# Ghostish/Open3DSOT

Hardware: NVIDIA H100
Metric: template-search pairs/sec, BAT-Car fwd+bwd (higher is better)
Workload: dtype f32

## Files before the change

### open3dsot_b200/csrc/common.cuh

```cuda
#pragma once
#include <cuda_runtime.h>
#include <stdint.h>

#define O3D_OK 0
#define O3D_ERR_ARG (-1)
#define O3D_ERR_ALIGN (-2)
#define O3D_ERR_CUDA (-3)

void o3d_set_error(const char* fmt, ...);

#define O3D_REQUIRE(cond, code, ...)                 \
    do {                                             \
        if (!(cond)) {                               \
            o3d_set_error(__VA_ARGS__);              \
            return (code);                           \
        }                                            \
    } while (0)

#define O3D_CHECK_LAUNCH(name)                                                        \
    do {                                                                              \
        cudaError_t e__ = cudaGetLastError();                                         \
        if (e__ != cudaSuccess) {                                                     \
            o3d_set_error("%s: launch failed: %s", name, cudaGetErrorString(e__));    \
            return O3D_ERR_CUDA;                                                      \
        }                                                                             \
    } while (0)

#define O3D_CUDA(call, name)                                                          \
    do {                                                                              \
        cudaError_t e__ = (call);                                                     \
        if (e__ != cudaSuccess) {                                                     \
            o3d_set_error("%s: %s", name, cudaGetErrorString(e__));                   \
            return O3D_ERR_CUDA;                                                      \
        }                                                                             \
    } while (0)

static inline int o3d_num_sms() {
    static int sms = 0;
    if (sms == 0) {
        int dev = 0;
        cudaGetDevice(&dev);
        cudaDeviceGetAttribute(&sms, cudaDevAttrMultiProcessorCount, dev);
        if (sms <= 0) sms = 132;
    }
    return sms;
}

static inline int o3d_opt_n_threads(int work) {
    if (work < 1) return 1;
    int p = 0;
    while ((1 << (p + 1)) <= work) ++p;
    int t = 1 << p;
    return t > 512 ? 512 : t;
}

#ifdef __CUDACC__
__device__ __forceinline__ float o3d_sq3(float dx, float dy, float dz) {
    return __fmaf_rn(dz, dz, __fmaf_rn(dy, dy, __fmul_rn(dx, dx)));
}
__device__ __forceinline__ float o3d_dist2(float ax, float ay, float az, float bx, float by, float bz) {
    return o3d_sq3(__fsub_rn(ax, bx), __fsub_rn(ay, by), __fsub_rn(az, bz));
}

__device__ __forceinline__ uint32_t o3d_smem_u32(const void* p) {
    return static_cast<uint32_t>(__cvta_generic_to_shared(p));
}
__device__ __forceinline__ void o3d_mbar_init(uint64_t* bar, uint32_t count) {
    asm volatile("mbarrier.init.shared::cta.b64 [%0], %1;" ::"r"(o3d_smem_u32(bar)), "r"(count));
}
__device__ __forceinline__ void o3d_fence_mbar_init() {
    asm volatile("fence.mbarrier_init.release.cluster;" ::: "memory");
}
__device__ __forceinline__ void o3d_fence_proxy_async() {
    asm volatile("fence.proxy.async.shared::cta;" ::: "memory");
}
__device__ __forceinline__ void o3d_mbar_expect_tx(uint64_t* bar, uint32_t bytes) {
    asm volatile("mbarrier.arrive.expect_tx.shared::cta.b64 _, [%0], %1;" ::"r"(o3d_smem_u32(bar)), "r"(bytes)
                 : "memory");
}
__device__ __forceinline__ void o3d_mbar_arrive(uint64_t* bar) {
    asm volatile("mbarrier.arrive.shared::cta.b64 _, [%0];" ::"r"(o3d_smem_u32(bar)) : "memory");
}
__device__ __forceinline__ bool o3d_mbar_try_wait(uint64_t* bar, uint32_t parity) {
    uint32_t ok;
    asm volatile(
        "{\n\t.reg .pred p;\n\t"
        "mbarrier.try_wait.parity.shared::cta.b64 p, [%1], %2;\n\t"
        "selp.u32 %0, 1, 0, p;\n\t}"
        : "=r"(ok)
        : "r"(o3d_smem_u32(bar)), "r"(parity)
        : "memory");
    return ok != 0;
}
__device__ __forceinline__ void o3d_mbar_wait(uint64_t* bar, uint32_t parity) {
    for (uint32_t spin = 0; spin < (1u << 28); ++spin)
        if (o3d_mbar_try_wait(bar, parity)) return;
    __trap();
}
__device__ __forceinline__ void o3d_bulk_g2s(void* smem_dst, const void* gsrc, uint32_t bytes, uint64_t* bar) {
    asm volatile(
        "cp.async.bulk.shared::cluster.global.mbarrier::complete_tx::bytes [%0], [%1], %2, [%3];" ::"r"(
            o3d_smem_u32(smem_dst)),
        "l"(gsrc), "r"(bytes), "r"(o3d_smem_u32(bar))
        : "memory");
}
__device__ __forceinline__ void o3d_prefetch_l2(const void* gptr, size_t bytes) {
    const char* p = static_cast<const char*>(gptr);
    const uintptr_t a = reinterpret_cast<uintptr_t>(p);
    const uintptr_t lo = a & ~(uintptr_t)15;
    size_t n = ((a - lo) + bytes + 15) & ~(size_t)15;
    const char* q = reinterpret_cast<const char*>(lo);
    while (n > 0) {
        const uint32_t c = n > (1u << 20) ? (1u << 20) : (uint32_t)n;
        asm volatile("cp.async.bulk.prefetch.L2.global [%0], %1;" ::"l"(q), "r"(c) : "memory");
        q += c;
        n -= c;
    }
}
__device__ __forceinline__ uint32_t o3d_block_exscan1024(uint32_t v, uint32_t* s_warp, uint32_t& total) {
    const int lane = threadIdx.x & 31, warp = threadIdx.x >> 5;
    uint32_t inc = v;
#pragma unroll
    for (int o = 1; o < 32; o <<= 1) {
        const uint32_t t = __shfl_up_sync(0xFFFFFFFFu, inc, o);
        if (lane >= o) inc += t;
    }
    if (lane == 31) s_warp[warp] = inc;
    __syncthreads();
    uint32_t w = s_warp[lane];
    uint32_t winc = w;
#pragma unroll
    for (int o = 1; o < 32; o <<= 1) {
        const uint32_t t = __shfl_up_sync(0xFFFFFFFFu, winc, o);
        if (lane >= o) winc += t;
    }
    total = __shfl_sync(0xFFFFFFFFu, winc, 31);
    const uint32_t wbase = __shfl_sync(0xFFFFFFFFu, winc - w, warp);
    __syncthreads();
    return wbase + inc - v;
}
__device__ __forceinline__ void o3d_to_box_frame(float dx, float dy, float dz, const float (&R)[9], float& x, float& y, float& z) {
    x = fmaf(dz, R[6], fmaf(dy, R[3], dx * R[0]));
    y = fmaf(dz, R[7], fmaf(dy, R[4], dx * R[1]));
    z = fmaf(dz, R[8], fmaf(dy, R[5], dx * R[2]));
}
__device__ __forceinline__ uint32_t o3d_lanemask_lt() {
    uint32_t m;
    asm("mov.u32 %0, %%lanemask_lt;" : "=r"(m));
    return m;
}
int o3d_pw_fwd_tc_dir(const float* x, int ldx, const float* in_scale, const float* in_shift, int in_relu, const void* wtiles,
                      const float* bias, int P, int K, int N, float* y, int ldy, double* sum, double* sumsq, int S, float* ymax,
                      float* ymin, int32_t* arg, int ldp, void* stream, bool reverse, bool bf16);
struct o3d_lift_t;
int o3d_pw_fwd_tc_lift_prec(const o3d_lift_t* lf, const int32_t* gidx, const float* in_scale, const float* in_shift, int in_relu,
                            const void* wtiles, const float* bias, int P, int K, int N, float* y, int ldy, double* sum,
                            double* sumsq, int S, float* ymax, float* ymin, int32_t* arg, int ldp, void* stream, bool bf16);
int o3d_pw_dgrad_tc_prec(const float* g, int ldg, const float* y, int ldy, const float* a, const float* b, const float* cc,
                         const float* dpool, const int32_t* sel, int S, int ldp, const void* wtiles_t, int P, int Cout, int Cin,
                         float* out, int ldo, const float* yprev, int ldyp, const float* pscale, const float* pshift, int prelu,
                         double* s1, double* s2y, void* stream, bool bf16);
int o3d_pw_dgrad_tc_lift_prec(const float* g, int ldg, const float* y, int ldy, const float* a, const float* b, const float* cc,
                              const float* dpool, const int32_t* sel, int S, int ldp, const void* wtiles_t, int P, int Cout,
                              int Cin, float* out, int ldo, const o3d_lift_t* lf, const int32_t* gidx, const float* pscale,
                              const float* pshift, int prelu, double* s1, double* s2y, void* stream, bool bf16);
int o3d_pw_wgrad_tc2_prec(const float* g, int ldg, const float* y, int ldy, const float* a, const float* b, const float* cc,
                          const float* dpool, const int32_t* sel, int S, int ldp, const float* x, int ldx, const float* in_scale,
                          const float* in_shift, int in_relu, int P, int Cout, int Cin, float* dw, int lddw, float* part,
                          long long part_floats, void* stream, bool bf16);
int o3d_pw_wgrad_tc_lift_prec(const float* g, int ldg, const float* y, int ldy, const float* a, const float* b, const float* cc,
                              const float* dpool, const int32_t* sel, int S, int ldp, const o3d_lift_t* lf, const int32_t* gidx,
                              const float* in_scale, const float* in_shift, int in_relu, int P, int Cout, int Cin, float* dw,
                              int lddw, float* part, long long part_floats, void* stream, bool bf16);
int o3d_pw_bwd_tc_prec(const float* g, int ldg, const float* y, int ldy, const float* a, const float* b, const float* cc,
                       const float* dpool, const int32_t* sel, int S, int ldp, const void* wtiles_t, const float* x,
                       const o3d_lift_t* lf, const int32_t* gidx, const float* in_scale, const float* in_shift, int in_relu, int P,
                       int Cout, int Cin, float* out, double* s1, double* s2y, float* dw, int lddw, float* part,
                       long long part_floats, void* stream, bool bf16);

#endif
```

### open3dsot_b200/csrc/lift.cu

```cuda
#include "common.cuh"
#include "lift.cuh"
#include "../../include/o3d_b200.h"

namespace {

constexpr int LIFT_THREADS = 256;

__device__ __forceinline__ float4 ldg4(const float* p) { return __ldg(reinterpret_cast<const float4*>(p)); }

struct LiftGeom { const int32_t* ridx; int ridx_mod, rows_per_cloud, pos_per_cloud; };

__device__ __forceinline__ int lift_row(const LiftGeom& g, int p) {
    const int cloud = p / g.pos_per_cloud;
    const int local = g.ridx ? __ldg(g.ridx + p) : (p % g.ridx_mod);
    return cloud * g.rows_per_cloud + local;
}

struct U4 { float4 u0, u1, u2, u3; };
__device__ __forceinline__ U4 load_u(const LiftView& lv, int c) {
    const float4 z = make_float4(0.f, 0.f, 0.f, 0.f);
    if (!lv.u) return U4{z, z, z, z};
    return U4{ldg4(lv.u + c), ldg4(lv.u + lv.ldz + c), ldg4(lv.u + 2 * lv.ldz + c), ldg4(lv.u + 3 * lv.ldz + c)};
}

template <bool STORE>
__global__ void __launch_bounds__(LIFT_THREADS, 4)
    lift_stats_kernel(LiftView lv, LiftGeom geo, int P, int C0, int grp, int32_t* __restrict__ gidx, float* __restrict__ y0,
                      double* __restrict__ sum, double* __restrict__ sumsq) {
    extern __shared__ double red[];
    const int tpr = C0 >> 2, rl = blockDim.x / tpr;
    const int t = threadIdx.x % tpr, lane = threadIdx.x / tpr;
    const int c = t * 4;
    const int n_groups = P / grp;
    const U4 u = load_u(lv, c);
    const float4 zero = make_float4(0.f, 0.f, 0.f, 0.f);
    if (!STORE && !sum) {
        if (lv.z && t == 0)
            for (int g = blockIdx.x * rl + lane; g < n_groups; g += gridDim.x * rl)
                for (int s = 0; s < grp; ++s) gidx[g * grp + s] = lift_row(geo, g * grp + s);
        return;
    }
    double d1[4] = {0.0, 0.0, 0.0, 0.0}, d2[4] = {0.0, 0.0, 0.0, 0.0};
    for (int g = blockIdx.x * rl + lane; g < n_groups; g += gridDim.x * rl) {
        float4 a1 = zero, a2 = zero;
        const int pb = g * grp;
#pragma unroll 4
        for (int s = 0; s < grp; ++s) {
            const int p = pb + s;
            float4 z4 = zero;
            if (lv.z) {
                const int row = lift_row(geo, p);
                if (t == 0) gidx[p] = row;
                z4 = ldg4(lv.z + (size_t)row * lv.ldz + c);
            }
            const float4 sv = lv.s ? ldg4(lv.s + (size_t)p * 4) : zero;
            const float4 v = lift_val4(z4, sv, u.u0, u.u1, u.u2, u.u3);
            if (STORE) *reinterpret_cast<float4*>(y0 + (size_t)p * lv.ldz + c) = v;
            a1.x += v.x; a1.y += v.y; a1.z += v.z; a1.w += v.w;
            a2.x = fmaf(v.x, v.x, a2.x); a2.y = fmaf(v.y, v.y, a2.y); a2.z = fmaf(v.z, v.z, a2.z); a2.w = fmaf(v.w, v.w, a2.w);
            if ((s & 31) == 31 || s == grp - 1) {
                d1[0] += a1.x; d1[1] += a1.y; d1[2] += a1.z; d1[3] += a1.w;
                d2[0] += a2.x; d2[1] += a2.y; d2[2] += a2.z; d2[3] += a2.w;
                a1 = a2 = zero;
            }
        }
    }
    if (!sum) return;
#pragma unroll
    for (int j = 0; j < 4; ++j) {
        red[(size_t)lane * C0 + c + j] = d1[j];
        red[(size_t)(rl + lane) * C0 + c + j] = d2[j];
    }
    __syncthreads();
    for (int ch = threadIdx.x; ch < C0; ch += blockDim.x) {
        double s1 = 0.0, s2 = 0.0;
        for (int l = 0; l < rl; ++l) { s1 += red[(size_t)l * C0 + ch]; s2 += red[(size_t)(rl + l) * C0 + ch]; }
        atomicAdd(sum + ch, s1);
        atomicAdd(sumsq + ch, s2);
    }
}

__global__ void __launch_bounds__(LIFT_THREADS, 4)
    lift_scatter_kernel(LiftView lv, int P, int C0, int grp, const float* __restrict__ y0, const float* __restrict__ g, int ldg,
                        const float* __restrict__ ca, const float* __restrict__ cb, const float* __restrict__ ccf,
                        float* __restrict__ dz, float* __restrict__ ds, float* __restrict__ du) {
    extern __shared__ float redf[];
    const int tpr = C0 >> 2, rl = blockDim.x / tpr;
    const int t = threadIdx.x % tpr, lane = threadIdx.x / tpr;
    const int c = t * 4;
    const int n_groups = P / grp;
    const U4 u = load_u(lv, c);
    const float4 one = make_float4(1.f, 1.f, 1.f, 1.f), zero = make_float4(0.f, 0.f, 0.f, 0.f);
    const float4 a4 = ca ? ldg4(ca + c) : one, b4 = ca ? ldg4(cb + c) : zero, k4 = ca ? ldg4(ccf + c) : zero;
    float4 du0 = zero, du1 = zero, du2 = zero, du3 = zero;
    const int w = tpr >= 32 ? 32 : tpr;
    const bool shfl = (tpr <= 32 && (tpr & (tpr - 1)) == 0) || (tpr % 32 == 0);
    for (int gb = blockIdx.x * rl; gb < n_groups; gb += gridDim.x * rl) {
        const bool valid = gb + lane < n_groups;
        const int gi = valid ? gb + lane : n_groups - 1;
        float4 acc0 = zero;
        const int pb = gi * grp;
        const int row0 = lv.z ? __ldg(lv.gidx + pb) : 0;
#pragma unroll 4
        for (int s = 0; s < grp; ++s) {
            const int p = pb + s;
            const int row = lv.z ? __ldg(lv.gidx + p) : 0;
            const float4 g4 = ldg4(g + (size_t)p * ldg + c);
            const float4 sv = lv.s ? ldg4(lv.s + (size_t)p * 4) : zero;
            float4 dy = g4;
            if (ca) {
                float4 v;
                if (y0) v = ldg4(y0 + (size_t)p * lv.ldz + c);
                else v = lift_val4(lv.z ? ldg4(lv.z + (size_t)row * lv.ldz + c) : zero, sv, u.u0, u.u1, u.u2, u.u3);
                dy.x = fmaf(a4.x, g4.x, fmaf(k4.x, v.x, b4.x)); dy.y = fmaf(a4.y, g4.y, fmaf(k4.y, v.y, b4.y));
                dy.z = fmaf(a4.z, g4.z, fmaf(k4.z, v.z, b4.z)); dy.w = fmaf(a4.w, g4.w, fmaf(k4.w, v.w, b4.w));
            }
            if (dz) {
                if (row == row0) { acc0.x += dy.x; acc0.y += dy.y; acc0.z += dy.z; acc0.w += dy.w; }
                else if (valid) atomicAdd(reinterpret_cast<float4*>(dz + (size_t)row * lv.ldz + c), dy);
            }
            if (du && valid) {
                du0.x = fmaf(sv.x, dy.x, du0.x); du0.y = fmaf(sv.x, dy.y, du0.y); du0.z = fmaf(sv.x, dy.z, du0.z); du0.w = fmaf(sv.x, dy.w, du0.w);
                du1.x = fmaf(sv.y, dy.x, du1.x); du1.y = fmaf(sv.y, dy.y, du1.y); du1.z = fmaf(sv.y, dy.z, du1.z); du1.w = fmaf(sv.y, dy.w, du1.w);
                du2.x = fmaf(sv.z, dy.x, du2.x); du2.y = fmaf(sv.z, dy.y, du2.y); du2.z = fmaf(sv.z, dy.z, du2.z); du2.w = fmaf(sv.z, dy.w, du2.w);
                du3.x = fmaf(sv.w, dy.x, du3.x); du3.y = fmaf(sv.w, dy.y, du3.y); du3.z = fmaf(sv.w, dy.z, du3.z); du3.w = fmaf(sv.w, dy.w, du3.w);
            }
            if (ds) {
                float4 d;
                d.x = fmaf(dy.x, u.u0.x, fmaf(dy.y, u.u0.y, fmaf(dy.z, u.u0.z, dy.w * u.u0.w)));
                d.y = fmaf(dy.x, u.u1.x, fmaf(dy.y, u.u1.y, fmaf(dy.z, u.u1.z, dy.w * u.u1.w)));
                d.z = fmaf(dy.x, u.u2.x, fmaf(dy.y, u.u2.y, fmaf(dy.z, u.u2.z, dy.w * u.u2.w)));
                d.w = fmaf(dy.x, u.u3.x, fmaf(dy.y, u.u3.y, fmaf(dy.z, u.u3.z, dy.w * u.u3.w)));
                if (shfl) {
                    for (int o = w >> 1; o >= 1; o >>= 1) {
                        d.x += __shfl_xor_sync(0xFFFFFFFFu, d.x, o, 32); d.y += __shfl_xor_sync(0xFFFFFFFFu, d.y, o, 32);
                        d.z += __shfl_xor_sync(0xFFFFFFFFu, d.z, o, 32); d.w += __shfl_xor_sync(0xFFFFFFFFu, d.w, o, 32);
                    }
                    if ((t & (w - 1)) == 0 && valid) atomicAdd(reinterpret_cast<float4*>(ds + (size_t)p * 4), d);
                } else if (valid) {
                    atomicAdd(reinterpret_cast<float4*>(ds + (size_t)p * 4), d);
                }
            }
        }
        if (dz && valid) atomicAdd(reinterpret_cast<float4*>(dz + (size_t)row0 * lv.ldz + c), acc0);
    }
    if (!du) return;
    float* r = redf + (size_t)lane * 4 * C0 + c;
    *reinterpret_cast<float4*>(r) = du0;
    *reinterpret_cast<float4*>(r + C0) = du1;
    *reinterpret_cast<float4*>(r + 2 * C0) = du2;
    *reinterpret_cast<float4*>(r + 3 * C0) = du3;
    __syncthreads();
    for (int e = threadIdx.x; e < 4 * C0; e += blockDim.x) {
        float s1 = 0.f;
        for (int l = 0; l < rl; ++l) s1 += redf[(size_t)l * 4 * C0 + e];
        atomicAdd(du + e, s1);
    }
}

int lift_check(const o3d_lift_t* lf, int P, int C0, const char* who) {
    O3D_REQUIRE(lf && (lf->z || lf->s), O3D_ERR_ARG, "%s: null lift descriptor (need z and / or s)", who);
    O3D_REQUIRE(C0 >= 4 && (C0 & 3) == 0 && C0 <= 1024 && lf->ldz == C0, O3D_ERR_ARG, "%s: C0=%d ldz=%d (need C0 %% 4 == 0, ldz == C0)",
                who, C0, lf->ldz);
    O3D_REQUIRE(lf->grp >= 1 && (lf->grp & (lf->grp - 1)) == 0 && P % lf->grp == 0, O3D_ERR_ARG,
                "%s: grp=%d must be a power of two dividing P=%d", who, lf->grp, P);
    O3D_REQUIRE(!lf->z || (lf->pos_per_cloud >= 1 && lf->rows_per_cloud >= 1 && (lf->ridx || lf->ridx_mod >= 1)), O3D_ERR_ARG,
                "%s: bad cloud geometry", who);
    O3D_REQUIRE(((uintptr_t)lf->s & 15) == 0 && ((uintptr_t)lf->u & 15) == 0 && ((uintptr_t)lf->z & 15) == 0, O3D_ERR_ALIGN,
                "%s: z / s / u must be 16-byte aligned", who);
    O3D_REQUIRE((lf->s == nullptr) == (lf->u == nullptr), O3D_ERR_ARG, "%s: s and u come together", who);
    return O3D_OK;
}

inline LiftView make_view(const o3d_lift_t* lf, const int32_t* gidx) {
    return LiftView{lf->z, lf->ldz, lf->z ? gidx : nullptr, lf->s, lf->u};
}

inline void lift_launch_shape(int P, int C0, int grp, int& threads, int& blocks, int& rl) {
    const int tpr = C0 / 4;
    rl = LIFT_THREADS / tpr;
    if (rl < 1) rl = 1;
    threads = tpr * rl;
    const int n_groups = P / grp;
    blocks = (n_groups + rl - 1) / rl;
    const int cap = 8 * o3d_num_sms();
    if (blocks > cap) blocks = cap;
    if (blocks < 1) blocks = 1;
}

}

extern "C" int o3d_lift_stats(const o3d_lift_t* lf, int P, int C0, int32_t* gidx, float* y0, double* sum, double* sumsq,
                              void* stream) {
    if (int e = lift_check(lf, P, C0, "o3d_lift_stats")) return e;
    O3D_REQUIRE(gidx || !lf->z, O3D_ERR_ARG, "o3d_lift_stats: gidx workspace missing");
    if (P == 0 || (!lf->z && !y0 && !sum)) return O3D_OK;
    int threads, blocks, rl;
    lift_launch_shape(P, C0, lf->grp, threads, blocks, rl);
    const LiftView lv = make_view(lf, gidx);
    const LiftGeom geo{lf->ridx, lf->ridx_mod, lf->rows_per_cloud, lf->pos_per_cloud};
    const size_t smem = sum ? sizeof(double) * 2 * rl * C0 : 0;
    cudaStream_t st = (cudaStream_t)stream;
    if (y0) lift_stats_kernel<true><<<blocks, threads, smem, st>>>(lv, geo, P, C0, lf->grp, gidx, y0, sum, sumsq);
    else lift_stats_kernel<false><<<blocks, threads, smem, st>>>(lv, geo, P, C0, lf->grp, gidx, y0, sum, sumsq);
    O3D_CHECK_LAUNCH("o3d_lift_stats");
    return O3D_OK;
}

extern "C" int o3d_lift_scatter(const o3d_lift_t* lf, int P, int C0, const int32_t* gidx, const float* y0, const float* g,
                                int ldg, const float* a, const float* b, const float* cc, void* stream) {
    if (int e = lift_check(lf, P, C0, "o3d_lift_scatter")) return e;
    O3D_REQUIRE((gidx || !lf->z) && g && (ldg & 3) == 0, O3D_ERR_ARG, "o3d_lift_scatter: null pointer / ldg");
    O3D_REQUIRE(!lf->d_s || lf->u, O3D_ERR_ARG, "o3d_lift_scatter: d_s without u");
    O3D_REQUIRE(((uintptr_t)lf->d_s & 15) == 0 && ((uintptr_t)lf->d_z & 15) == 0, O3D_ERR_ALIGN, "o3d_lift_scatter: alignment");
    if (P == 0) return O3D_OK;
    int threads, blocks, rl;
    lift_launch_shape(P, C0, lf->grp, threads, blocks, rl);
    const LiftView lv = make_view(lf, gidx);
    const size_t smem = (lf->s && lf->d_u) ? sizeof(float) * rl * 4 * C0 : 0;
    lift_scatter_kernel<<<blocks, threads, smem, (cudaStream_t)stream>>>(lv, P, C0, lf->grp, y0, g, ldg, a, b, cc,
                                                                        lf->z ? lf->d_z : nullptr, lf->s ? lf->d_s : nullptr,
                                                                        lf->s ? lf->d_u : nullptr);
    O3D_CHECK_LAUNCH("o3d_lift_scatter");
    return O3D_OK;
}
```

### open3dsot_b200/csrc/lift.cuh

```cuda
#pragma once
#include <stdint.h>

struct LiftView {
    const float* z; int ldz;
    const int32_t* gidx;
    const float* s;
    const float* u;
};

#ifdef __CUDACC__
__device__ __forceinline__ float lift_val(float z, const float4& s, float u0, float u1, float u2, float u3) {
    return fmaf(s.w, u3, fmaf(s.z, u2, fmaf(s.y, u1, fmaf(s.x, u0, z))));
}
__device__ __forceinline__ float4 lift_val4(const float4& z, const float4& s, const float4& u0, const float4& u1, const float4& u2,
                                            const float4& u3) {
    return make_float4(lift_val(z.x, s, u0.x, u1.x, u2.x, u3.x), lift_val(z.y, s, u0.y, u1.y, u2.y, u3.y),
                       lift_val(z.z, s, u0.z, u1.z, u2.z, u3.z), lift_val(z.w, s, u0.w, u1.w, u2.w, u3.w));
}
#endif
```

### open3dsot_b200/csrc/pwmlp_tc.cu

```cuda
#include <type_traits>
#include "common.cuh"
#include "lift.cuh"
#include "tc_ptx.cuh"
#include "../../include/o3d_b200.h"

namespace {

struct TcAct {
    const float* x; int ld; const float* scale; const float* shift; int relu;
    struct Coef { float4 s, t; bool on; };
    template <int R> struct Batch { float4 v[R]; };
    __device__ __forceinline__ Coef prep(int k, int K) const {
        Coef c;
        c.on = k < K;
        c.s = make_float4(1.f, 1.f, 1.f, 1.f);
        c.t = make_float4(0.f, 0.f, 0.f, 0.f);
        if (c.on && scale) { c.s = ld4g(scale + k); c.t = ld4g(shift + k); }
        return c;
    }
    template <int R>
    __device__ __forceinline__ void fetch(Batch<R>& b, int p0, int stride, int P, int k, int K) const {
        const int kk = k < K ? k : 0;
#pragma unroll
        for (int i = 0; i < R; ++i) {
            const int p = p0 + i * stride;
            b.v[i] = ld4g(x + (size_t)(p < P ? p : P - 1) * ld + kk);
        }
    }
    template <int R>
    __device__ __forceinline__ float4 finish(const Batch<R>& b, const Coef& c, int i, int p, int P) const {
        float4 v = b.v[i];
        if (!(c.on && p < P)) return make_float4(0.f, 0.f, 0.f, 0.f);
        if (scale) { v.x = fmaf(v.x, c.s.x, c.t.x); v.y = fmaf(v.y, c.s.y, c.t.y); v.z = fmaf(v.z, c.s.z, c.t.z); v.w = fmaf(v.w, c.s.w, c.t.w); }
        if (relu) { v.x = fmaxf(v.x, 0.f); v.y = fmaxf(v.y, 0.f); v.z = fmaxf(v.z, 0.f); v.w = fmaxf(v.w, 0.f); }
        return v;
    }
    __device__ __forceinline__ void prefetch_rows(int p0, int rows, int P) const {
        if (p0 < P) o3d_prefetch_l2(x + (size_t)p0 * ld, (size_t)min(rows, P - p0) * ld * sizeof(float));
    }
};

struct TcLift {
    LiftView lv; const float* scale; const float* shift; int relu;
    int la;
    struct Coef { float4 s, t, u0, u1, u2, u3; bool on; };
    template <int R> struct Batch { float4 v[R]; float4 sv[R]; int nrow[R]; int tag; };
    __device__ __forceinline__ Coef prep(int k, int K) const {
        Coef c;
        c.on = k < K;
        c.s = make_float4(1.f, 1.f, 1.f, 1.f);
        c.t = c.u0 = c.u1 = c.u2 = c.u3 = make_float4(0.f, 0.f, 0.f, 0.f);
        if (c.on && scale) { c.s = ld4g(scale + k); c.t = ld4g(shift + k); }
        if (c.on && lv.u) { c.u0 = ld4g(lv.u + k); c.u1 = ld4g(lv.u + lv.ldz + k); c.u2 = ld4g(lv.u + 2 * lv.ldz + k); c.u3 = ld4g(lv.u + 3 * lv.ldz + k); }
        return c;
    }
    template <int R>
    __device__ __forceinline__ void fetch(Batch<R>& b, int p0, int stride, int P, int k, int K) const {
        const int kk = k < K ? k : 0;
        if (lv.z) {
            int row[R];
            if (b.tag == p0 + 1) {
#pragma unroll
                for (int i = 0; i < R; ++i) row[i] = b.nrow[i];
            } else if (R == 4 && stride == 1 && (p0 & 3) == 0 && p0 + 3 < P) {
                const int4 r4 = __ldg(reinterpret_cast<const int4*>(lv.gidx + p0));
                row[0] = r4.x; row[R > 1 ? 1 : 0] = r4.y; row[R > 2 ? 2 : 0] = r4.z; row[R > 3 ? 3 : 0] = r4.w;
            } else {
#pragma unroll
                for (int i = 0; i < R; ++i) {
                    const int p = p0 + i * stride;
                    row[i] = __ldg(lv.gidx + (p < P ? p : P - 1));
                }
            }
#pragma unroll
            for (int i = 0; i < R; ++i) b.v[i] = ld4g(lv.z + (size_t)row[i] * lv.ldz + kk);
            if (la == 0) {
#pragma unroll
                for (int i = 0; i < R; ++i) b.nrow[i] = row[i];
                b.tag = p0 + 1;
            } else {
                const int pn = p0 + la;
#pragma unroll
                for (int i = 0; i < R; ++i) {
                    const int p = pn + i * stride;
                    b.nrow[i] = __ldg(lv.gidx + (p < P ? p : P - 1));
                }
                b.tag = pn + 1;
            }
        }
        if (lv.s) {
#pragma unroll
            for (int i = 0; i < R; ++i) {
                const int p = p0 + i * stride;
                b.sv[i] = ld4g(lv.s + (size_t)(p < P ? p : P - 1) * 4);
            }
        }
    }
    template <int R>
    __device__ __forceinline__ float4 finish(const Batch<R>& b, const Coef& c, int i, int p, int P) const {
        const float4 zero = make_float4(0.f, 0.f, 0.f, 0.f);
        if (!(c.on && p < P)) return zero;
        float4 v = lift_val4(lv.z ? b.v[i] : zero, lv.s ? b.sv[i] : zero, c.u0, c.u1, c.u2, c.u3);
        if (scale) { v.x = fmaf(v.x, c.s.x, c.t.x); v.y = fmaf(v.y, c.s.y, c.t.y); v.z = fmaf(v.z, c.s.z, c.t.z); v.w = fmaf(v.w, c.s.w, c.t.w); }
        if (relu) { v.x = fmaxf(v.x, 0.f); v.y = fmaxf(v.y, 0.f); v.z = fmaxf(v.z, 0.f); v.w = fmaxf(v.w, 0.f); }
        return v;
    }
    __device__ __forceinline__ void prefetch_rows(int p0, int rows, int P) const {
        if (p0 >= P) return;
        const size_t n = (size_t)min(rows, P - p0);
        if (lv.z) o3d_prefetch_l2(lv.gidx + p0, n * sizeof(int32_t));
        if (lv.s) o3d_prefetch_l2(lv.s + (size_t)p0 * 4, n * 16);
    }
};

struct TcDy {
    const float* g; int ldg; const float* y; int ldy; const float* a; const float* b; const float* cc;
    const float* dpool; const int32_t* sel; int S; int ldp;
    int sh;
    struct Coef { float4 a, b, c; bool on; };
    template <int R> struct Batch { float4 g[R]; float4 y[R]; bool shared; };
    __device__ __forceinline__ Coef prep(int k, int K) const {
        Coef c;
        c.on = k < K;
        c.a = make_float4(1.f, 1.f, 1.f, 1.f);
        c.b = c.c = make_float4(0.f, 0.f, 0.f, 0.f);
        if (c.on && a) { c.a = ld4g(a + k); c.b = ld4g(b + k); c.c = ld4g(cc + k); }
        return c;
    }
    template <int R>
    __device__ __forceinline__ void fetch(Batch<R>& bt, int p0, int stride, int P, int k, int K) const {
        const int kk = k < K ? k : 0;
        bt.shared = false;
        if (dpool) {
            const int pf = p0 < P ? p0 : P - 1;
            const int pe = p0 + (R - 1) * stride;
            const int pl = pe < P ? pe : P - 1;
            if (R >= 2 && (pf >> sh) == (pl >> sh)) {
                bt.shared = true;
                const size_t go = (size_t)(pf >> sh) * ldp + kk;
                bt.g[0] = ld4g(dpool + go);
                const int4 sl = __ldg(reinterpret_cast<const int4*>(sel + go));
                bt.g[R >= 2 ? 1 : 0] = make_float4(__int_as_float(sl.x), __int_as_float(sl.y), __int_as_float(sl.z), __int_as_float(sl.w));
            } else {
#pragma unroll
                for (int i = 0; i < R; ++i) {
                    const int p = p0 + i * stride, pp = p < P ? p : P - 1;
                    const int s = pp & (S - 1);
                    const size_t go = (size_t)(pp >> sh) * ldp + kk;
                    const int4 sl = __ldg(reinterpret_cast<const int4*>(sel + go));
                    const float4 d = ld4g(dpool + go);
                    bt.g[i] = make_float4(sl.x == s ? d.x : 0.f, sl.y == s ? d.y : 0.f, sl.z == s ? d.z : 0.f, sl.w == s ? d.w : 0.f);
                }
            }
        } else {
#pragma unroll
            for (int i = 0; i < R; ++i) {
                const int p = p0 + i * stride;
                bt.g[i] = ld4g(g + (size_t)(p < P ? p : P - 1) * ldg + kk);
            }
        }
#pragma unroll
        for (int i = 0; i < R; ++i) {
            const int p = p0 + i * stride;
            bt.y[i] = a ? ld4g(y + (size_t)(p < P ? p : P - 1) * ldy + kk) : make_float4(0.f, 0.f, 0.f, 0.f);
        }
    }
    template <int R>
    __device__ __forceinline__ float4 finish(const Batch<R>& bt, const Coef& c, int i, int p, int P) const {
        if (!(c.on && p < P)) return make_float4(0.f, 0.f, 0.f, 0.f);
        float4 v = bt.g[i];
        if (bt.shared) {
            const int s = p & (S - 1);
            const float4 d = bt.g[0], sl = bt.g[R >= 2 ? 1 : 0];
            v = make_float4(__float_as_int(sl.x) == s ? d.x : 0.f, __float_as_int(sl.y) == s ? d.y : 0.f,
                            __float_as_int(sl.z) == s ? d.z : 0.f, __float_as_int(sl.w) == s ? d.w : 0.f);
        }
        if (a) {
            const float4 yy = bt.y[i];
            v.x = fmaf(c.a.x, v.x, fmaf(c.c.x, yy.x, c.b.x)); v.y = fmaf(c.a.y, v.y, fmaf(c.c.y, yy.y, c.b.y));
            v.z = fmaf(c.a.z, v.z, fmaf(c.c.z, yy.z, c.b.z)); v.w = fmaf(c.a.w, v.w, fmaf(c.c.w, yy.w, c.b.w));
        }
        return v;
    }
    __device__ __forceinline__ void prefetch_rows(int p0, int rows, int P) const {
        if (p0 >= P) return;
        const size_t n = (size_t)min(rows, P - p0);
        if (!dpool) o3d_prefetch_l2(g + (size_t)p0 * ldg, n * ldg * sizeof(float));
        if (a) o3d_prefetch_l2(y + (size_t)p0 * ldy, n * ldy * sizeof(float));
        if (dpool) {
            const int g0 = p0 >> sh, g1 = (p0 + (int)n - 1) >> sh;
            const size_t bytes = (size_t)(g1 - g0 + 1) * ldp * sizeof(float);
            o3d_prefetch_l2(dpool + (size_t)g0 * ldp, bytes);
            o3d_prefetch_l2(sel + (size_t)g0 * ldp, bytes);
        }
    }
};

template <class L> struct Bf16 : L {};
template <class L> struct is_bf16 { static constexpr bool value = false; };
template <class L> struct is_bf16<Bf16<L>> { static constexpr bool value = true; };
template <class L> struct is_lift { static constexpr bool value = std::is_same<L, TcLift>::value; };
template <class L> struct is_lift<Bf16<L>> { static constexpr bool value = is_lift<L>::value; };

template <int LD>
struct TcFwdEpi {
    float* y; int ldy; const float* bias; double* sum; double* sumsq;
    int S, log2S; float* ymax; float* ymin; int32_t* arg; int ldp;
    float bv, mx, mn; int ax, an; double d1, d2;
    __device__ __forceinline__ void begin(int ch, int Nw) {
        d1 = d2 = 0.0;
        bv = (bias && ch < Nw) ? bias[ch] : 0.f;
        mx = -INFINITY; mn = INFINITY; ax = an = 0;
    }
    __device__ __forceinline__ void prefetch(int, int, int, int) {}
    __device__ __forceinline__ const int32_t* lift_gidx() const { return nullptr; }
    __device__ __forceinline__ const float* lift_s() const { return nullptr; }
    __device__ __forceinline__ void set_tile(const int32_t*, const float4*) {}
    __device__ __forceinline__ void group(const uint32_t (&r)[16], int ch, int Nw, int pbase, int P) {
        if (ch >= Nw) return;
        float s1 = 0.f, s2 = 0.f;
        const int smask = S - 1;
        float* yp = y ? y + (size_t)pbase * ldy + ch : nullptr;
        if (pbase + 16 <= P && (S == 0 || S >= 16)) {
            float v[16];
#pragma unroll
            for (int j = 0; j < 16; ++j) v[j] = __uint_as_float(r[j]) + bv;
            if (yp) {
                const size_t st = LD ? (size_t)LD : (size_t)ldy;
#pragma unroll
                for (int j = 0; j < 16; ++j) yp[j * st] = v[j];
            }
#pragma unroll
            for (int j = 0; j < 16; ++j) {
                s1 += v[j];
                s2 = fmaf(v[j], v[j], s2);
            }
            if (S > 0) {
                float gm = v[0], gn = v[0];
                int ga = 0, gb = 0;
#pragma unroll
                for (int j = 1; j < 16; ++j) {
                    if (v[j] > gm) { gm = v[j]; ga = j; }
                    if (v[j] < gn) { gn = v[j]; gb = j; }
                }
                const int s0 = pbase & smask;
                if (s0 == 0) { mx = gm; ax = ga; mn = gn; an = gb; }
                else {
                    if (gm > mx) { mx = gm; ax = s0 + ga; }
                    if (gn < mn) { mn = gn; an = s0 + gb; }
                }
                if (s0 + 16 == S) {
                    const size_t o = (size_t)(pbase >> log2S) * ldp + ch;
                    ymax[o] = mx; ymin[o] = mn; arg[o] = ax | (an << 16);
                }
            }
        } else {
#pragma unroll
            for (int j = 0; j < 16; ++j) {
                if (pbase + j >= P) break;
                const float v = __uint_as_float(r[j]) + bv;
                if (yp) yp[(size_t)j * ldy] = v;
                s1 += v;
                s2 = fmaf(v, v, s2);
                if (S > 0) {
                    const int s = (pbase + j) & smask;
                    if (s == 0) { mx = -INFINITY; mn = INFINITY; ax = an = 0; }
                    if (v > mx) { mx = v; ax = s; }
                    if (v < mn) { mn = v; an = s; }
                    if (s == smask) {
                        const size_t o = (size_t)((pbase + j) >> log2S) * ldp + ch;
                        ymax[o] = mx; ymin[o] = mn; arg[o] = ax | (an << 16);
                    }
                }
            }
        }
        d1 += (double)s1;
        d2 += (double)s2;
    }
    __device__ __forceinline__ void end(int ch, int Nw) {
        if (sum && ch < Nw) {
            atomicAdd(sum + ch, d1);
            atomicAdd(sumsq + ch, d2);
        }
    }
};

template <int LD, bool LIFT = false>
struct TcDgradEpi {
    float* out; int ldo; const float* yprev; int ldyp; const float* scale; const float* shift; int relu;
    double* s1g; double* s2y;
    LiftView lv;
    float sc, sh; double d1, d2;
    float yv[16];
    float u0, u1, u2, u3; const int32_t* gs; const float4* ss;
    __device__ __forceinline__ bool lifted() const { return LIFT; }
    __device__ __forceinline__ void begin(int ch, int Nw) {
        d1 = d2 = 0.0;
        sc = (scale && ch < Nw) ? scale[ch] : 1.f;
        sh = (shift && ch < Nw) ? shift[ch] : 0.f;
        if constexpr (LIFT) {
            const bool on = lv.u && ch < Nw;
            u0 = on ? lv.u[ch] : 0.f; u1 = on ? lv.u[lv.ldz + ch] : 0.f; u2 = on ? lv.u[2 * lv.ldz + ch] : 0.f; u3 = on ? lv.u[3 * lv.ldz + ch] : 0.f;
            gs = nullptr;
        }
    }
    __device__ __forceinline__ const int32_t* lift_gidx() const { return LIFT ? lv.gidx : nullptr; }
    __device__ __forceinline__ const float* lift_s() const { return LIFT ? lv.s : nullptr; }
    __device__ __forceinline__ void set_tile(const int32_t* g, const float4* s4) { if constexpr (LIFT) { gs = g; ss = s4; } }
    __device__ __forceinline__ void prefetch_lift(int ch, int pbase, int col, int P) {
#pragma unroll
        for (int j = 0; j < 16; ++j) {
            const float z = lv.z ? __ldg(lv.z + (size_t)gs[col + j] * lv.ldz + ch) : 0.f;
            const float4 sv = lv.s ? ss[col + j] : make_float4(0.f, 0.f, 0.f, 0.f);
            yv[j] = lift_val(z, sv, u0, u1, u2, u3);
        }
    }
    __device__ __forceinline__ void prefetch(int ch, int Nw, int pbase, int P) {
        if (ch >= Nw) return;
        if constexpr (LIFT) { prefetch_lift(ch, pbase, pbase & (TC_N - 1), P); return; }
        if (!yprev) return;
        if (pbase + 16 <= P) {
            const float* yp = yprev + (size_t)pbase * ldyp + ch;
            const size_t st = LD ? (size_t)LD : (size_t)ldyp;
#pragma unroll
            for (int j = 0; j < 16; ++j) yv[j] = __ldg(yp + j * st);
        } else {
#pragma unroll
            for (int j = 0; j < 16; ++j) {
                const int pj = min(pbase + j, P - 1);
                yv[j] = __ldg(yprev + (size_t)pj * ldyp + ch);
            }
        }
    }
    __device__ __forceinline__ void group(const uint32_t (&r)[16], int ch, int Nw, int pbase, int P) {
        if (ch >= Nw) return;
        float s1 = 0.f, s2 = 0.f;
        float* op = out + (size_t)pbase * ldo + ch;
        if (pbase + 16 <= P) {
            float v[16];
#pragma unroll
            for (int j = 0; j < 16; ++j) v[j] = __uint_as_float(r[j]);
            if (yprev || lifted()) {
                if (relu) {
#pragma unroll
                    for (int j = 0; j < 16; ++j) v[j] = fmaf(yv[j], sc, sh) > 0.f ? v[j] : 0.f;
                }
#pragma unroll
                for (int j = 0; j < 16; ++j) s2 = fmaf(v[j], yv[j], s2);
            }
            const size_t st = LD ? (size_t)LD : (size_t)ldo;
#pragma unroll
            for (int j = 0; j < 16; ++j) {
                s1 += v[j];
                op[j * st] = v[j];
            }
        } else {
#pragma unroll
            for (int j = 0; j < 16; ++j) {
                if (pbase + j >= P) break;
                float v = __uint_as_float(r[j]);
                if (yprev || lifted()) {
                    if (relu && !(fmaf(yv[j], sc, sh) > 0.f)) v = 0.f;
                    s2 = fmaf(v, yv[j], s2);
                }
                s1 += v;
                op[(size_t)j * ldo] = v;
            }
        }
        d1 += (double)s1;
        d2 += (double)s2;
    }
    __device__ __forceinline__ void end(int ch, int Nw) {
        if (s1g && ch < Nw) {
            atomicAdd(s1g + ch, d1);
            atomicAdd(s2y + ch, d2);
        }
    }
};

constexpr int TC_STAGES = 2;
constexpr int TC_STAGE_BYTES = 4 * TILE_BYTES;
constexpr int TC_EPI_LD = 68;
constexpr int TC_EPI_BYTES = TC_M * TC_EPI_LD * 4;
constexpr int TC_THREADS = 512;
constexpr int TC_SMEM = TC_STAGES * TC_STAGE_BYTES + 2 * TC_EPI_BYTES + 1024 + 256 + 1024 + 4096;

template <int R>
__device__ __forceinline__ void stage_acc(const float (&acc)[R], float* stg, int ld) {
    const int w = (threadIdx.x >> 5) & 3, lane = threadIdx.x & 31;
#pragma unroll
    for (int i = 0; i < R; ++i) {
        const int row = 16 * w + (lane >> 2) + 8 * ((i >> 1) & 1), col = 8 * (i >> 2) + 2 * (lane & 3) + (i & 1);
        stg[col * ld + row] = acc[i];
    }
}

template <class BLoad, class Epi>
__global__ void __launch_bounds__(TC_THREADS, 1)
    pw_tc_kernel(BLoad bl, const uint8_t* __restrict__ wtiles, int P, int K, int Nw, int nkb, Epi epi, int rev) {
    constexpr bool BF = is_bf16<BLoad>::value;
    constexpr int WBYTES = BF ? BF_TILE_BYTES : 2 * TILE_BYTES;
    extern __shared__ uint8_t smem_raw[];
    uint8_t* smem = reinterpret_cast<uint8_t*>((reinterpret_cast<uintptr_t>(smem_raw) + 1023) & ~(uintptr_t)1023);
    uint8_t* tail = smem + TC_STAGES * TC_STAGE_BYTES + 2 * TC_EPI_BYTES;
    uint64_t* full = reinterpret_cast<uint64_t*>(tail);
    uint64_t* empty = full + TC_STAGES;

    const int warp = threadIdx.x >> 5, lane = threadIdx.x & 31;
    const int mt0 = blockIdx.y;
    const int n_ptiles = (P + TC_N - 1) / TC_N;
    auto tile_of = [&](int t) { return rev ? n_ptiles - 1 - t : t; };

    if (threadIdx.x == 0) {
        for (int s = 0; s < TC_STAGES; ++s) {
            o3d_mbar_init(full + s, 256 + 1);
            o3d_mbar_init(empty + s, 8);
        }
        o3d_fence_mbar_init();
    }
    __syncthreads();

    if (warp < 8) {
        const int h = warp >> 2;
        const int tw = threadIdx.x & 127;
        const int ch = mt0 * TC_M + tw;
        float* stg = reinterpret_cast<float*>(smem + TC_STAGES * TC_STAGE_BYTES + h * TC_EPI_BYTES);
        int32_t* gsm = reinterpret_cast<int32_t*>(tail + 256);
        float4* ssm = reinterpret_cast<float4*>(tail + 256 + 1024);
        epi.begin(ch, Nw);
        int stage = 0, phase = 0, buf = 0;
        for (int t = blockIdx.x; t < n_ptiles; t += gridDim.x) {
            const int pt0 = tile_of(t) * TC_N;
            {
                const int32_t* gi = epi.lift_gidx();
                const float* si = epi.lift_s();
                if (gi || si) {
                    const int pp = min(pt0 + tw, P - 1);
                    if (gi && h == 0) gsm[buf * TC_N + tw] = __ldg(gi + pp);
                    if (si && h == 1) ssm[buf * TC_N + tw] = ld4g(si + (size_t)pp * 4);
                    asm volatile("bar.sync 1, 256;" ::: "memory");
                    epi.set_tile(gsm + buf * TC_N, ssm + buf * TC_N);
                }
            }
            const int pb = pt0 + h * 64;
            epi.prefetch(ch, Nw, pb, P);
            float acc[64];
#pragma unroll
            for (int i = 0; i < 64; ++i) acc[i] = 0.f;
            for (int kb = 0; kb < nkb; ++kb) {
                o3d_mbar_wait(full + stage, phase);
                const uint32_t sb = o3d_smem_u32(smem + stage * TC_STAGE_BYTES);
                wgmma_fence_acc(acc);
                wgmma_fence();
                if constexpr (BF) {
                    const uint32_t xb = sb + 2 * TILE_BYTES + h * (BF_TILE_BYTES / 2);
                    wgmma_bf16_kblock<128>(acc, make_desc_sw64(xb), make_desc_sw64(sb), kb == 0);
                } else {
                    const uint32_t xb = sb + 2 * TILE_BYTES + h * (TILE_BYTES / 2);
                    wgmma_3xtf32_kblock<128>(acc, make_desc(xb), make_desc(xb + TILE_BYTES), make_desc(sb), make_desc(sb + TILE_BYTES),
                                             kb == 0);
                }
                wgmma_commit();
                wgmma_wait<0>();
                wgmma_fence_acc(acc);
                if (lane == 0) o3d_mbar_arrive(empty + stage);
                if (++stage == TC_STAGES) { stage = 0; phase ^= 1; }
            }
            asm volatile("bar.sync %0, 128;" ::"r"(2 + h) : "memory");
            stage_acc(acc, stg, TC_EPI_LD);
            asm volatile("bar.sync %0, 128;" ::"r"(2 + h) : "memory");
            const float* row = stg + tw * TC_EPI_LD;
#pragma unroll 1
            for (int cg = 0; cg < 4; ++cg) {
                uint32_t r[16];
#pragma unroll
                for (int j = 0; j < 4; ++j) {
                    const float4 v = *reinterpret_cast<const float4*>(row + cg * 16 + 4 * j);
                    r[4 * j] = __float_as_uint(v.x); r[4 * j + 1] = __float_as_uint(v.y);
                    r[4 * j + 2] = __float_as_uint(v.z); r[4 * j + 3] = __float_as_uint(v.w);
                }
                epi.group(r, ch, Nw, pb + cg * 16, P);
                if (cg + 1 < 4) epi.prefetch(ch, Nw, pb + (cg + 1) * 16, P);
            }
            buf ^= 1;
        }
        epi.end(ch, Nw);
    } else {
        const int pt = (warp - 8) * 32 + lane;
        const int chunk = pt & 7;
        const int row0 = (pt >> 3) * 4;
        int stage = 0, phase = 0;
        struct Cur { int t, kb, p0; };
        auto advance = [&](Cur& c) {
            if (++c.kb == nkb) {
                c.kb = 0;
                c.t += gridDim.x;
                if (c.t < n_ptiles) c.p0 = tile_of(c.t) * TC_N;
            }
        };
        using Batch4 = typename BLoad::template Batch<4>;
        auto issue = [&](Batch4& r, typename BLoad::Coef& cf, const Cur& c) {
            if (c.t >= n_ptiles) return;
            const int k = c.kb * TC_K + chunk * 4;
            cf = bl.prep(k, K);
            bl.fetch(r, c.p0 + row0, 1, P, k, K);
        };
        Cur c0{(int)blockIdx.x, 0, 0};
        if (c0.t < n_ptiles) c0.p0 = tile_of(c0.t) * TC_N;
        Batch4 r0{};
        typename BLoad::Coef f0 = bl.prep(chunk * 4, K);
        issue(r0, f0, c0);
        if (pt == 0 && c0.t < n_ptiles) bl.prefetch_rows(c0.p0, TC_N, P);
        while (c0.t < n_ptiles) {
            o3d_mbar_wait(empty + stage, phase ^ 1);
            if (pt == 0) {
                o3d_mbar_expect_tx(full + stage, WBYTES);
                o3d_bulk_g2s(smem + stage * TC_STAGE_BYTES, wtiles + ((size_t)mt0 * nkb + c0.kb) * WBYTES, WBYTES, full + stage);
                const int tn = c0.t + (int)gridDim.x;
                if (c0.kb == 0 && tn < n_ptiles) bl.prefetch_rows(tile_of(tn) * TC_N, TC_N, P);
            }
            uint8_t* xhi = smem + stage * TC_STAGE_BYTES + 2 * TILE_BYTES;
            uint8_t* xlo = xhi + TILE_BYTES;
#pragma unroll
            for (int i = 0; i < 4; ++i) {
                const float4 v = bl.finish(r0, f0, i, c0.p0 + row0 + i, P);
                if constexpr (BF) {
                    *reinterpret_cast<uint2*>(xhi + sw64(row0 + i, chunk >> 1) + (chunk & 1) * 8) = pack_bf16x4(v);
                } else {
                    const uint32_t off = sw128(row0 + i, chunk);
                    *reinterpret_cast<float4*>(xhi + off) = hi_part(v);
                    *reinterpret_cast<float4*>(xlo + off) = lo_part(v);
                }
            }
            o3d_fence_proxy_async();
            o3d_mbar_arrive(full + stage);
            if (++stage == TC_STAGES) { stage = 0; phase ^= 1; }
            advance(c0);
            issue(r0, f0, c0);
        }
    }
}

constexpr int WG_STAGES = 3;
constexpr int WG_AHEAD = 4;
constexpr int WG_THREADS = 512;
constexpr int WG_SMEM = WG_STAGES * 4 * TILE_BYTES + 1024 + 256;

template <class L>
__device__ __forceinline__ void store_transposed(const L& ld, const typename L::template Batch<4>& raw, const typename L::Coef& cf,
                                                 uint8_t* hi, int c_local, int p_first, int prow0, int pend) {
#pragma unroll
    for (int i = 0; i < 4; ++i) {
        const int pl = prow0 + 8 * i;
        const float4 v = ld.finish(raw, cf, i, p_first + pl, pend);
        const float e[4] = {v.x, v.y, v.z, v.w};
#pragma unroll
        for (int j = 0; j < 4; ++j) {
            const uint32_t off = sw128(c_local + j, pl >> 2) + (uint32_t)((pl & 3) * 4);
            const float h = hi1(e[j]);
            *reinterpret_cast<float*>(hi + off) = h;
            *reinterpret_cast<float*>(hi + TILE_BYTES + off) = e[j] - h;
        }
    }
}

constexpr int WG_BF_SUB = TC_K * TC_BF_ROW;
constexpr int WG_BF_X = 4 * WG_BF_SUB;

template <class L>
__device__ __forceinline__ void store_rows_bf16(const L& ld, const typename L::template Batch<4>& raw, const typename L::Coef& cf,
                                                uint8_t* img, int sub, int c_local, int p_first, int prow0, int pend) {
#pragma unroll
    for (int i = 0; i < 4; ++i) {
        const int pl = prow0 + 8 * i;
        st_bf16_row4(img, sub, pl, c_local, ld.finish(raw, cf, i, p_first + pl, pend));
    }
}

template <class XB>
__global__ void __launch_bounds__(WG_THREADS, 1)
    pw_wgrad_tc_kernel(TcDy da, XB xb, int P, int M, int N, int chunk, float* __restrict__ part) {
    constexpr bool BF = is_bf16<XB>::value;
    extern __shared__ uint8_t smem_raw[];
    uint8_t* smem = reinterpret_cast<uint8_t*>((reinterpret_cast<uintptr_t>(smem_raw) + 1023) & ~(uintptr_t)1023);
    uint64_t* full = reinterpret_cast<uint64_t*>(smem + WG_STAGES * 4 * TILE_BYTES);
    uint64_t* empty = full + WG_STAGES;

    const int warp = threadIdx.x >> 5, lane = threadIdx.x & 31;
    const int m0 = blockIdx.z * TC_M, n0 = blockIdx.y * TC_N;
    const int pbeg = blockIdx.x * chunk, pend = min(P, pbeg + chunk);
    const int nkb = pend > pbeg ? (pend - pbeg + TC_K - 1) / TC_K : 0;
    auto kpos = [&](int i) { return pbeg + i * TC_K; };

    if (threadIdx.x == 0) {
        for (int s = 0; s < WG_STAGES; ++s) {
            o3d_mbar_init(full + s, 256);
            o3d_mbar_init(empty + s, 8);
        }
        o3d_fence_mbar_init();
    }
    __syncthreads();

    if (warp < 8) {
        const int h = warp >> 2, w = warp & 3;
        float acc[64];
#pragma unroll
        for (int i = 0; i < 64; ++i) acc[i] = 0.f;
        int stage = 0, phase = 0;
        for (int kb = 0; kb < nkb; ++kb) {
            o3d_mbar_wait(full + stage, phase);
            const uint32_t sb = o3d_smem_u32(smem + stage * 4 * TILE_BYTES);
            wgmma_fence_acc(acc);
            wgmma_fence();
            if constexpr (BF) {
                const uint32_t ab = sb + h * 2 * WG_BF_SUB;
#pragma unroll
                for (int ks = 0; ks < 2; ++ks)
                    wgmma_bf16_tt_n128(acc, make_desc_sw64_mn(ab + ks * 1024, WG_BF_SUB),
                                       make_desc_sw64_mn(sb + WG_BF_X + ks * 1024, WG_BF_SUB), (kb == 0 && ks == 0) ? 0u : 1u);
            } else {
                const uint32_t ab = sb + h * (TILE_BYTES / 2);
                wgmma_3xtf32_kblock<128>(acc, make_desc(ab), make_desc(ab + TILE_BYTES), make_desc(sb + 2 * TILE_BYTES),
                                         make_desc(sb + 3 * TILE_BYTES), kb == 0);
            }
            wgmma_commit();
            wgmma_wait<0>();
            wgmma_fence_acc(acc);
            if (lane == 0) o3d_mbar_arrive(empty + stage);
            if (++stage == WG_STAGES) { stage = 0; phase ^= 1; }
        }
        const int Mt = TC_M * (int)gridDim.z, Nt = TC_N * (int)gridDim.y;
        float* __restrict__ out = part + (size_t)blockIdx.x * Mt * Nt;
#pragma unroll
        for (int i = 0; i < 64; i += 4) {
#pragma unroll
            for (int rr = 0; rr < 2; ++rr) {
                const int m = m0 + h * 64 + 16 * w + (lane >> 2) + 8 * rr, n = n0 + 8 * (i >> 2) + 2 * (lane & 3);
                *reinterpret_cast<float2*>(out + (size_t)m * Nt + n) = make_float2(acc[i + 2 * rr], acc[i + 2 * rr + 1]);
            }
        }
    } else {
        const int pw = warp - 8;
        const int c4 = pw * 4 + (lane & 3), prow0 = lane >> 2;
        const bool pt0 = pw == 0 && lane == 0;
        TcDy::Batch<4> ra = {};
        typename XB::template Batch<4> rb = {};
        auto fetch = [&](int kb) {
            da.fetch(ra, kpos(kb) + prow0, 8, pend, m0 + c4 * 4, M);
            xb.fetch(rb, kpos(kb) + prow0, 8, pend, n0 + c4 * 4, N);
        };
        auto prefetch = [&](int kb) {
            if (pt0 && kb < nkb) {
                da.prefetch_rows(kpos(kb), TC_K, pend);
                xb.prefetch_rows(kpos(kb), TC_K, pend);
            }
        };
        int stage = 0, phase = 0;
        for (int kb = 0; kb < WG_AHEAD; ++kb) prefetch(kb);
        if (nkb > 0) fetch(0);
        for (int kb = 0; kb < nkb; ++kb) {
            prefetch(kb + WG_AHEAD);
            o3d_mbar_wait(empty + stage, phase ^ 1);
            uint8_t* sbase = smem + stage * 4 * TILE_BYTES;
            if constexpr (BF) {
                store_rows_bf16(da, ra, da.prep(m0 + c4 * 4, M), sbase, WG_BF_SUB, c4 * 4, kpos(kb), prow0, pend);
                store_rows_bf16(xb, rb, xb.prep(n0 + c4 * 4, N), sbase + WG_BF_X, WG_BF_SUB, c4 * 4, kpos(kb), prow0, pend);
            } else {
                store_transposed(da, ra, da.prep(m0 + c4 * 4, M), sbase, c4 * 4, kpos(kb), prow0, pend);
                store_transposed(xb, rb, xb.prep(n0 + c4 * 4, N), sbase + 2 * TILE_BYTES, c4 * 4, kpos(kb), prow0, pend);
            }
            o3d_fence_proxy_async();
            o3d_mbar_arrive(full + stage);
            if (kb + 1 < nkb) fetch(kb + 1);
            if (++stage == WG_STAGES) { stage = 0; phase ^= 1; }
        }
    }
}

__global__ void __launch_bounds__(256)
    wgrad_reduce_kernel(const float* __restrict__ part, int splits, int Mt, int Nt, int M, int N, float* __restrict__ dW,
                        int lddw) {
    const int sub = threadIdx.x & 7;
    const int n4 = (blockIdx.x * 32 + (threadIdx.x >> 3)) * 4, m = blockIdx.y;
    float4 acc = make_float4(0.f, 0.f, 0.f, 0.f);
    if (n4 < N && m < M) {
        const float* p = part + (size_t)m * Nt + n4;
        for (int s = sub; s < splits; s += 8) {
            const float4 v = __ldg(reinterpret_cast<const float4*>(p + (size_t)s * Mt * Nt));
            acc.x += v.x; acc.y += v.y; acc.z += v.z; acc.w += v.w;
        }
    }
#pragma unroll
    for (int o = 4; o >= 1; o >>= 1) {
        acc.x += __shfl_xor_sync(0xFFFFFFFFu, acc.x, o); acc.y += __shfl_xor_sync(0xFFFFFFFFu, acc.y, o);
        acc.z += __shfl_xor_sync(0xFFFFFFFFu, acc.z, o); acc.w += __shfl_xor_sync(0xFFFFFFFFu, acc.w, o);
    }
    if (sub == 0 && n4 < N && m < M) {
        float* o = dW + (size_t)m * lddw + n4;
        o[0] += acc.x;
        if (n4 + 1 < N) o[1] += acc.y;
        if (n4 + 2 < N) o[2] += acc.z;
        if (n4 + 3 < N) o[3] += acc.w;
    }
}

constexpr int BW_TP = 64;
constexpr int BW_THREADS = 384;
constexpr int BW_DY = 0, BW_XT = 64 * 1024, BW_W = 128 * 1024, BW_TAIL = 192 * 1024;
constexpr int BW_SMEM = BW_TAIL + 256 + 1024 + 4096 + 1024;
constexpr int BW_BF_SUB = BW_TP * TC_BF_ROW;

template <class XB, int N>
__global__ void __launch_bounds__(BW_THREADS, 1)
    pw_bwd_tc_kernel(TcDy da, XB xb, const uint8_t* __restrict__ wtiles, int P, int M, TcDgradEpi<N, is_lift<XB>::value> epi,
                     float* __restrict__ part) {
    constexpr bool BF = is_bf16<XB>::value;
    constexpr int NH = N / 2;
    constexpr int WSTAGE = BF ? NH * TC_BF_ROW : 2 * NH * 128;
    extern __shared__ uint8_t smem_raw[];
    uint8_t* smem = reinterpret_cast<uint8_t*>((reinterpret_cast<uintptr_t>(smem_raw) + 1023) & ~(uintptr_t)1023);
    uint8_t* tail = smem + BW_TAIL;
    uint64_t* dy_full = reinterpret_cast<uint64_t*>(tail);
    uint64_t* dy_empty = dy_full + 1;
    uint64_t* xt_full = dy_full + 2;
    uint64_t* xt_empty = dy_full + 3;
    uint64_t* wfull = dy_full + 4;

    const int warp = threadIdx.x >> 5, lane = threadIdx.x & 31;
    const int nkb = M / TC_K;
    const int n_ptiles = (P + BW_TP - 1) / BW_TP;
    const int my_tiles = blockIdx.x < n_ptiles ? (n_ptiles - 1 - blockIdx.x) / gridDim.x + 1 : 0;

    if (threadIdx.x == 0) {
        o3d_mbar_init(dy_full, 128);
        o3d_mbar_init(dy_empty, 8);
        o3d_mbar_init(xt_full, 128);
        o3d_mbar_init(xt_empty, 8);
        for (int s = 0; s < 4; ++s) o3d_mbar_init(wfull + s, 1);
        o3d_fence_mbar_init();
    }
    __syncthreads();

    if (warp < 8) {
        const int h = warp >> 2, w = warp & 3, tw = threadIdx.x & 127;
        uint8_t* wring = smem + BW_W + h * 2 * WSTAGE;
        const int n_witems = my_tiles * nkb;
        auto load_w = [&](int item) {
            const int s = item & 1;
            o3d_mbar_expect_tx(wfull + 2 * h + s, WSTAGE);
            if constexpr (BF) {
                const uint8_t* src = wtiles + (size_t)(item % nkb) * BF_TILE_BYTES + h * NH * TC_BF_ROW;
                o3d_bulk_g2s(wring + s * WSTAGE, src, WSTAGE, wfull + 2 * h + s);
            } else {
                const uint8_t* src = wtiles + (size_t)(item % nkb) * (2 * TILE_BYTES) + h * NH * 128;
                o3d_bulk_g2s(wring + s * WSTAGE, src, NH * 128, wfull + 2 * h + s);
                o3d_bulk_g2s(wring + s * WSTAGE + NH * 128, src + TILE_BYTES, NH * 128, wfull + 2 * h + s);
            }
        };
        if (tw == 0) {
            if (n_witems > 0) load_w(0);
            if (n_witems > 1) load_w(1);
        }
        const bool do_w = 64 * h < M;
        const int n_local = h * NH + (tw % NH);
        const int q = tw / NH;
        constexpr int PPT = NH / 2;
        float* stg = reinterpret_cast<float*>(smem + BW_XT + h * (NH * TC_EPI_LD * 4));
        int32_t* gsm = reinterpret_cast<int32_t*>(tail + 256);
        float4* ssm = reinterpret_cast<float4*>(tail + 256 + 1024);
        epi.begin(n_local, N);
        float wacc[N / 2];
#pragma unroll
        for (int i = 0; i < N / 2; ++i) wacc[i] = 0.f;
        int witem = 0, tphase = 0, buf = 0;
        for (int t = blockIdx.x; t < n_ptiles; t += gridDim.x) {
            const int pt0 = t * BW_TP;
            {
                const int32_t* gi = epi.lift_gidx();
                const float* si = epi.lift_s();
                if (gi || si) {
                    if (tw < BW_TP) {
                        const int pp = min(pt0 + tw, P - 1);
                        const int slot = buf * TC_N + ((pt0 + tw) & (TC_N - 1));
                        if (gi && h == 0) gsm[slot] = __ldg(gi + pp);
                        if (si && h == 1) ssm[slot] = ld4g(si + (size_t)pp * 4);
                    }
                    asm volatile("bar.sync 1, 256;" ::: "memory");
                    epi.set_tile(gsm + buf * TC_N, ssm + buf * TC_N);
                }
            }
            const int pb = pt0 + q * PPT;
            float dacc[NH / 2];
#pragma unroll
            for (int i = 0; i < NH / 2; ++i) dacc[i] = 0.f;
            o3d_mbar_wait(dy_full, tphase);
            for (int kb = 0; kb < nkb; ++kb, ++witem) {
                o3d_mbar_wait(wfull + 2 * h + (witem & 1), (witem >> 1) & 1);
                const uint32_t bb = o3d_smem_u32(wring + (witem & 1) * WSTAGE);
                wgmma_fence_acc(dacc);
                wgmma_fence();
                if constexpr (BF) {
                    wgmma_bf16_kblock<NH>(dacc, make_desc_sw64(o3d_smem_u32(smem + BW_DY + kb * BW_BF_SUB)), make_desc_sw64(bb), kb == 0);
                } else {
                    const uint32_t ab = o3d_smem_u32(smem + BW_DY + kb * TILE_BYTES);
                    wgmma_3xtf32_kblock<NH>(dacc, make_desc(ab), make_desc(ab + TILE_BYTES / 2), make_desc(bb), make_desc(bb + NH * 128),
                                            kb == 0);
                }
                wgmma_commit();
                wgmma_wait<0>();
                wgmma_fence_acc(dacc);
                asm volatile("bar.sync %0, 128;" ::"r"(2 + h) : "memory");
                if (tw == 0 && witem + 2 < n_witems) load_w(witem + 2);
            }
            o3d_mbar_wait(xt_full, tphase);
            if constexpr (BF) {
                if (do_w) {
                    const uint32_t ab = o3d_smem_u32(smem + BW_DY + 2 * h * BW_BF_SUB), xb0 = o3d_smem_u32(smem + BW_XT);
                    wgmma_fence_acc(wacc);
                    wgmma_fence();
#pragma unroll
                    for (int ks = 0; ks < BW_TP / 16; ++ks) {
                        const uint64_t ad = make_desc_sw64_mn(ab + ks * 1024, BW_BF_SUB), bd = make_desc_sw64_mn(xb0 + ks * 1024, BW_BF_SUB);
                        if constexpr (N == 128) wgmma_bf16_tt_n128(wacc, ad, bd, 1u);
                        else wgmma_bf16_tt_n64(wacc, ad, bd, 1u);
                    }
                    wgmma_commit();
                    wgmma_wait<0>();
                    wgmma_fence_acc(wacc);
                }
            } else if (do_w) {
                const int mr = 16 * w + (lane >> 2);
                const uint8_t* dyk = smem + BW_DY + (2 * h + (w >> 1)) * (TILE_BYTES);
                const int mc = mr & 31;
                const uint32_t xt = o3d_smem_u32(smem + BW_XT);
#pragma unroll 1
                for (int ks = 0; ks < BW_TP / 8; ++ks) {
                    uint32_t ahi[4], alo[4];
#pragma unroll
                    for (int i = 0; i < 4; ++i) {
                        const int p = ks * 8 + (lane & 3) + 4 * (i >> 1), m = mc + 8 * (i & 1);
                        const uint32_t off = sw128(p, m >> 2) + 4 * (m & 3);
                        ahi[i] = *reinterpret_cast<const uint32_t*>(dyk + off);
                        alo[i] = *reinterpret_cast<const uint32_t*>(dyk + TILE_BYTES / 2 + off);
                    }
                    const uint32_t xb0 = xt + (ks >> 2) * (2 * TILE_BYTES) + (ks & 3) * 32;
                    const uint64_t bhi = make_desc(xb0), blo = make_desc(xb0 + TILE_BYTES);
                    wgmma_fence_acc(wacc);
                    wgmma_fence();
                    if constexpr (N == 128) {
                        wgmma_tf32_rs_n128(wacc, alo, bhi);
                        wgmma_tf32_rs_n128(wacc, ahi, blo);
                        wgmma_tf32_rs_n128(wacc, ahi, bhi);
                    } else {
                        wgmma_tf32_rs_n64(wacc, alo, bhi);
                        wgmma_tf32_rs_n64(wacc, ahi, blo);
                        wgmma_tf32_rs_n64(wacc, ahi, bhi);
                    }
                    wgmma_commit();
                    wgmma_wait<0>();
                    wgmma_fence_acc(wacc);
                }
            }
            __syncwarp();
            if (lane == 0) o3d_mbar_arrive(dy_empty);
            epi.prefetch(n_local, N, pb, P);
            asm volatile("bar.sync 4, 256;" ::: "memory");
            stage_acc(dacc, stg, TC_EPI_LD);
            asm volatile("bar.sync %0, 128;" ::"r"(2 + h) : "memory");
            const float* row = stg + (tw % NH) * TC_EPI_LD + q * PPT;
#pragma unroll 1
            for (int cg = 0; cg < PPT / 16; ++cg) {
                uint32_t r[16];
#pragma unroll
                for (int j = 0; j < 4; ++j) {
                    const float4 v = *reinterpret_cast<const float4*>(row + cg * 16 + 4 * j);
                    r[4 * j] = __float_as_uint(v.x); r[4 * j + 1] = __float_as_uint(v.y);
                    r[4 * j + 2] = __float_as_uint(v.z); r[4 * j + 3] = __float_as_uint(v.w);
                }
                epi.group(r, n_local, N, pb + cg * 16, P);
                if (cg + 1 < PPT / 16) epi.prefetch(n_local, N, pb + (cg + 1) * 16, P);
            }
            __syncwarp();
            if (lane == 0) o3d_mbar_arrive(xt_empty);
            tphase ^= 1;
            buf ^= 1;
        }
        epi.end(n_local, N);
        if (do_w) {
            float* __restrict__ out = part + (size_t)blockIdx.x * TC_M * TC_N;
#pragma unroll
            for (int i = 0; i < N / 2; i += 4) {
#pragma unroll
                for (int rr = 0; rr < 2; ++rr) {
                    const int m = 64 * h + 16 * w + (lane >> 2) + 8 * rr, n = 8 * (i >> 2) + 2 * (lane & 3);
                    *reinterpret_cast<float2*>(out + (size_t)m * TC_N + n) = make_float2(wacc[i + 2 * rr], wacc[i + 2 * rr + 1]);
                }
            }
        }
    } else {
        const int pt = threadIdx.x - 256;
        const int chunk = pt & 7, row0 = (pt >> 3) * 4;
        const int pw = warp - 8, c4 = pw * 4 + (lane & 3), prow0 = lane >> 2;
        constexpr int NXH = N / 64;
        const int n_items_x = 2 * NXH;
        struct It { int t, i; };
        TcDy::Batch<4> ra{};
        typename XB::template Batch<4> rb{};
        It ca{(int)blockIdx.x, 0}, cb{(int)blockIdx.x, 0};
        auto fetch_a = [&](const It& c) {
            if (c.t < n_ptiles) da.fetch(ra, c.t * BW_TP + row0, 1, P, c.i * TC_K + chunk * 4, M);
        };
        auto fetch_b = [&](const It& c) {
            if (c.t < n_ptiles)
                xb.fetch(rb, c.t * BW_TP + (c.i >> (NXH - 1)) * TC_K + prow0, 8, P, (c.i & (NXH - 1)) * 64 + c4 * 4, N);
        };
        fetch_a(ca);
        fetch_b(cb);
        if (pt == 0 && ca.t < n_ptiles) { da.prefetch_rows(ca.t * BW_TP, BW_TP, P); xb.prefetch_rows(ca.t * BW_TP, BW_TP, P); }
        int tphase = 0;
        for (int t = blockIdx.x; t < n_ptiles; t += gridDim.x) {
            const int pt0 = t * BW_TP;
            if (pt == 0) {
                const int tn = t + (int)gridDim.x;
                if (tn < n_ptiles) { da.prefetch_rows(tn * BW_TP, BW_TP, P); xb.prefetch_rows(tn * BW_TP, BW_TP, P); }
            }
            o3d_mbar_wait(dy_empty, tphase ^ 1);
            for (int kb = 0; kb < nkb; ++kb) {
                const int k = kb * TC_K + chunk * 4;
                const TcDy::Coef cf = da.prep(k, M);
                if constexpr (BF) {
#pragma unroll
                    for (int i = 0; i < 4; ++i)
                        st_bf16_row4(smem + BW_DY + kb * BW_BF_SUB, 0, row0 + i, chunk * 4, da.finish(ra, cf, i, pt0 + row0 + i, P));
                } else {
                    uint8_t* hi = smem + BW_DY + kb * TILE_BYTES;
#pragma unroll
                    for (int i = 0; i < 4; ++i) {
                        const float4 v = da.finish(ra, cf, i, pt0 + row0 + i, P);
                        const uint32_t off = sw128(row0 + i, chunk);
                        *reinterpret_cast<float4*>(hi + off) = hi_part(v);
                        *reinterpret_cast<float4*>(hi + TILE_BYTES / 2 + off) = lo_part(v);
                    }
                }
                if (++ca.i == nkb) { ca.i = 0; ca.t += gridDim.x; }
                fetch_a(ca);
            }
            o3d_fence_proxy_async();
            o3d_mbar_arrive(dy_full);
            o3d_mbar_wait(xt_empty, tphase ^ 1);
            for (int it = 0; it < n_items_x; ++it) {
                const int j = it >> (NXH - 1), cl = (it & (NXH - 1)) * 64 + c4 * 4;
                if constexpr (BF)
                    store_rows_bf16(xb, rb, xb.prep(cl, N), smem + BW_XT + j * (TC_K * TC_BF_ROW), BW_BF_SUB, cl, pt0 + j * TC_K, prow0, P);
                else
                    store_transposed(xb, rb, xb.prep(cl, N), smem + BW_XT + j * (2 * TILE_BYTES), cl, pt0 + j * TC_K, prow0, P);
                if (++cb.i == n_items_x) { cb.i = 0; cb.t += gridDim.x; }
                fetch_b(cb);
            }
            o3d_fence_proxy_async();
            o3d_mbar_arrive(xt_full);
            tphase ^= 1;
        }
    }
}

__global__ void w_pretile_kernel(const float* __restrict__ W, int ld, int rows, int K, int nkb, uint8_t* __restrict__ out) {
    const int m_tile = blockIdx.y, kb = blockIdx.x;
    uint8_t* dst = out + ((size_t)m_tile * nkb + kb) * (2 * TILE_BYTES);
    for (int id = threadIdx.x; id < TC_M * 8; id += blockDim.x) {
        const int r = id >> 3, c = id & 7;
        const int row = m_tile * TC_M + r, k = kb * TC_K + c * 4;
        float4 v = make_float4(0.f, 0.f, 0.f, 0.f);
        if (row < rows && k < K) v = *reinterpret_cast<const float4*>(W + (size_t)row * ld + k);
        const uint32_t off = sw128(r, c);
        *reinterpret_cast<float4*>(dst + off) = hi_part(v);
        *reinterpret_cast<float4*>(dst + TILE_BYTES + off) = lo_part(v);
    }
}

inline int ilog2_exact(int v) { int l = 0; while ((1 << l) < v) ++l; return l; }

template <class BLoad, class Epi>
int launch_tc(BLoad bl, const uint8_t* wtiles, int P, int K, int Nw, Epi epi, bool reverse, cudaStream_t st, const char* name) {
    auto kern = pw_tc_kernel<BLoad, Epi>;
    O3D_CUDA(cudaFuncSetAttribute(kern, cudaFuncAttributeMaxDynamicSharedMemorySize, TC_SMEM), name);
    const int gy = (Nw + TC_M - 1) / TC_M;
    const int nkb = (K + TC_K - 1) / TC_K;
    const int n_ptiles = (P + TC_N - 1) / TC_N;
    int gx = o3d_num_sms() / gy;
    if (gx < 1) gx = 1;
    if (gx > n_ptiles) gx = n_ptiles;
    kern<<<dim3(gx, gy), TC_THREADS, TC_SMEM, st>>>(bl, wtiles, P, K, Nw, nkb, epi, reverse);
    O3D_CHECK_LAUNCH(name);
    return O3D_OK;
}

template <int LD, class BLoad>
int launch_fwd(const BLoad& bl, const void* wtiles, const float* bias, int P, int K, int Nw, float* y, int ldy, double* sum,
               double* sumsq, int S, float* ymax, float* ymin, int32_t* arg, int ldp, bool reverse, cudaStream_t st) {
    TcFwdEpi<LD> ep{};
    ep.y = y; ep.ldy = ldy; ep.bias = bias; ep.sum = sum; ep.sumsq = sumsq;
    ep.S = S; ep.ymax = ymax; ep.ymin = ymin; ep.arg = arg; ep.ldp = ldp;
    ep.log2S = 0;
    while ((1 << ep.log2S) < S) ++ep.log2S;
    return launch_tc(bl, (const uint8_t*)wtiles, P, K, Nw, ep, reverse, st, "o3d_pw_fwd_tc");
}

template <int LD, bool LIFT = false, class BL>
int launch_dgrad(const BL& bl, const void* wtiles_t, int P, int Cout, int Cin, float* out, int ldo, const float* yprev,
                 int ldyp, const float* pscale, const float* pshift, int prelu, double* s1, double* s2y, cudaStream_t st,
                 const LiftView* lv = nullptr) {
    if constexpr (!LIFT) {
        if (lv) return launch_dgrad<LD, true>(bl, wtiles_t, P, Cout, Cin, out, ldo, yprev, ldyp, pscale, pshift, prelu, s1, s2y, st, lv);
    }
    TcDgradEpi<LD, LIFT> ep{};
    if (lv) ep.lv = *lv;
    ep.out = out; ep.ldo = ldo; ep.yprev = yprev; ep.ldyp = ldyp; ep.scale = pscale; ep.shift = pshift; ep.relu = prelu;
    ep.s1g = s1; ep.s2y = s2y;
    return launch_tc(bl, (const uint8_t*)wtiles_t, P, Cout, Cin, ep, false, st, "o3d_pw_dgrad_tc");
}

}

extern "C" long long o3d_pw_tc_wtile_bytes(int rows, int K) {
    const long long mt = (rows + TC_M - 1) / TC_M, nkb = (K + TC_K - 1) / TC_K;
    return mt * nkb * 2 * TILE_BYTES;
}

extern "C" int o3d_pw_tc_pretile(const float* w, int ldw, int rows, int K, void* wtiles, void* stream) {
    O3D_REQUIRE(w && wtiles, O3D_ERR_ARG, "o3d_pw_tc_pretile: null pointer");
    O3D_REQUIRE((K & 3) == 0 && (ldw & 3) == 0, O3D_ERR_ARG, "o3d_pw_tc_pretile: K and ldw must be multiples of 4");
    O3D_REQUIRE(((uintptr_t)wtiles & 15) == 0 && ((uintptr_t)w & 15) == 0, O3D_ERR_ALIGN, "o3d_pw_tc_pretile: alignment");
    const int mt = (rows + TC_M - 1) / TC_M, nkb = (K + TC_K - 1) / TC_K;
    w_pretile_kernel<<<dim3(nkb, mt), 256, 0, (cudaStream_t)stream>>>(w, ldw, rows, K, nkb, (uint8_t*)wtiles);
    O3D_CHECK_LAUNCH("o3d_pw_tc_pretile");
    return O3D_OK;
}

int o3d_pw_fwd_tc_dir(const float* x, int ldx, const float* in_scale, const float* in_shift, int in_relu, const void* wtiles,
                      const float* bias, int P, int K, int N, float* y, int ldy, double* sum, double* sumsq, int S, float* ymax,
                      float* ymin, int32_t* arg, int ldp, void* stream, bool reverse, bool bf16) {
    O3D_REQUIRE(x && wtiles, O3D_ERR_ARG, "o3d_pw_fwd_tc: null pointer");
    O3D_REQUIRE(P >= 0 && K >= 4 && N >= 1 && (K & 3) == 0 && (ldx & 3) == 0, O3D_ERR_ARG, "o3d_pw_fwd_tc: bad sizes");
    O3D_REQUIRE(S == 0 || (P % S == 0 && 64 % S == 0 && ymax && ymin && arg), O3D_ERR_ARG,
                "o3d_pw_fwd_tc: pooling group size must divide 64 and P");
    if (P == 0) return O3D_OK;
    const int Nw = (N + 3) & ~3;
    TcAct bl{x, ldx, in_scale, in_shift, in_relu};
    cudaStream_t st = (cudaStream_t)stream;
    if (bf16) {
        Bf16<TcAct> bb{bl};
#define O3D_FWD_ARGS bb, wtiles, bias, P, K, Nw, y, ldy, sum, sumsq, S, ymax, ymin, arg, ldp, reverse, st
        if (ldy == 64) return launch_fwd<64>(O3D_FWD_ARGS);
        if (ldy == 128) return launch_fwd<128>(O3D_FWD_ARGS);
        if (ldy == 256) return launch_fwd<256>(O3D_FWD_ARGS);
        return launch_fwd<0>(O3D_FWD_ARGS);
#undef O3D_FWD_ARGS
    }
#define O3D_FWD_ARGS bl, wtiles, bias, P, K, Nw, y, ldy, sum, sumsq, S, ymax, ymin, arg, ldp, reverse, st
    if (ldy == 64) return launch_fwd<64>(O3D_FWD_ARGS);
    if (ldy == 128) return launch_fwd<128>(O3D_FWD_ARGS);
    if (ldy == 256) return launch_fwd<256>(O3D_FWD_ARGS);
    return launch_fwd<0>(O3D_FWD_ARGS);
#undef O3D_FWD_ARGS
}

extern "C" int o3d_pw_fwd_tc(const float* x, int ldx, const float* in_scale, const float* in_shift, int in_relu,
                             const void* wtiles, const float* bias, int P, int K, int N, float* y, int ldy, double* sum,
                             double* sumsq, int S, float* ymax, float* ymin, int32_t* arg, int ldp, void* stream) {
    return o3d_pw_fwd_tc_dir(x, ldx, in_scale, in_shift, in_relu, wtiles, bias, P, K, N, y, ldy, sum, sumsq, S, ymax, ymin, arg,
                             ldp, stream, false, false);
}

namespace {
int dgrad_tc_impl(const float* g, int ldg, const float* y, int ldy, const float* a, const float* b, const float* cc,
                  const float* dpool, const int32_t* sel, int S, int ldp, const void* wtiles_t, int P, int Cout, int Cin,
                  float* out, int ldo, const float* yprev, int ldyp, const float* pscale, const float* pshift, int prelu,
                  double* s1, double* s2y, void* stream, const LiftView* lv, bool bf16) {
    O3D_REQUIRE((g || dpool) && wtiles_t && out, O3D_ERR_ARG, "o3d_pw_dgrad_tc: null pointer");
    O3D_REQUIRE((Cout & 3) == 0 && (Cin & 3) == 0, O3D_ERR_ARG, "o3d_pw_dgrad_tc: channel counts must be multiples of 4");
    if (P == 0) return O3D_OK;
    TcDy bl{g, ldg, y, ldy, a, b, cc, dpool, sel, S > 0 ? S : 1, ldp, ilog2_exact(S > 0 ? S : 1)};
    cudaStream_t st = (cudaStream_t)stream;
    const int ld = (!yprev || ldyp == ldo) ? ldo : 0;
    auto run = [&](const auto& ldr) {
#define O3D_DG_ARGS ldr, wtiles_t, P, Cout, Cin, out, ldo, yprev, ldyp, pscale, pshift, prelu, s1, s2y, st, lv
        if (ld == 64) return launch_dgrad<64>(O3D_DG_ARGS);
        if (ld == 128) return launch_dgrad<128>(O3D_DG_ARGS);
        if (ld == 256) return launch_dgrad<256>(O3D_DG_ARGS);
        return launch_dgrad<0>(O3D_DG_ARGS);
#undef O3D_DG_ARGS
    };
    return bf16 ? run(Bf16<TcDy>{bl}) : run(bl);
}
}

int o3d_pw_dgrad_tc_prec(const float* g, int ldg, const float* y, int ldy, const float* a, const float* b, const float* cc,
                         const float* dpool, const int32_t* sel, int S, int ldp, const void* wtiles_t, int P, int Cout, int Cin,
                         float* out, int ldo, const float* yprev, int ldyp, const float* pscale, const float* pshift, int prelu,
                         double* s1, double* s2y, void* stream, bool bf16) {
    return dgrad_tc_impl(g, ldg, y, ldy, a, b, cc, dpool, sel, S, ldp, wtiles_t, P, Cout, Cin, out, ldo, yprev, ldyp, pscale,
                         pshift, prelu, s1, s2y, stream, nullptr, bf16);
}

extern "C" int o3d_pw_dgrad_tc(const float* g, int ldg, const float* y, int ldy, const float* a, const float* b,
                               const float* cc, const float* dpool, const int32_t* sel, int S, int ldp,
                               const void* wtiles_t, int P, int Cout, int Cin, float* out, int ldo, const float* yprev,
                               int ldyp, const float* pscale, const float* pshift, int prelu, double* s1, double* s2y,
                               void* stream) {
    return dgrad_tc_impl(g, ldg, y, ldy, a, b, cc, dpool, sel, S, ldp, wtiles_t, P, Cout, Cin, out, ldo, yprev, ldyp, pscale,
                         pshift, prelu, s1, s2y, stream, nullptr, false);
}

int o3d_pw_dgrad_tc_lift_prec(const float* g, int ldg, const float* y, int ldy, const float* a, const float* b, const float* cc,
                              const float* dpool, const int32_t* sel, int S, int ldp, const void* wtiles_t, int P, int Cout,
                              int Cin, float* out, int ldo, const o3d_lift_t* lf, const int32_t* gidx, const float* pscale,
                              const float* pshift, int prelu, double* s1, double* s2y, void* stream, bool bf16) {
    O3D_REQUIRE(lf && (gidx || !lf->z) && (lf->z || lf->s) && lf->ldz == Cin, O3D_ERR_ARG, "o3d_pw_dgrad_tc_lift: lift descriptor");
    const LiftView lv{lf->z, lf->ldz, lf->z ? gidx : nullptr, lf->s, lf->u};
    return dgrad_tc_impl(g, ldg, y, ldy, a, b, cc, dpool, sel, S, ldp, wtiles_t, P, Cout, Cin, out, ldo, nullptr, 0, pscale,
                         pshift, prelu, s1, s2y, stream, &lv, bf16);
}

extern "C" int o3d_pw_dgrad_tc_lift(const float* g, int ldg, const float* y, int ldy, const float* a, const float* b,
                                    const float* cc, const float* dpool, const int32_t* sel, int S, int ldp,
                                    const void* wtiles_t, int P, int Cout, int Cin, float* out, int ldo,
                                    const o3d_lift_t* lf, const int32_t* gidx, const float* pscale, const float* pshift,
                                    int prelu, double* s1, double* s2y, void* stream) {
    return o3d_pw_dgrad_tc_lift_prec(g, ldg, y, ldy, a, b, cc, dpool, sel, S, ldp, wtiles_t, P, Cout, Cin, out, ldo, lf, gidx, pscale,
                                     pshift, prelu, s1, s2y, stream, false);
}

namespace {
template <class XB>
int launch_wgrad(const TcDy& da, const XB& xb, int P, int Cout, int Cin, float* dw, int lddw, float* part, long long part_floats,
                 cudaStream_t st) {
    auto kern = pw_wgrad_tc_kernel<XB>;
    O3D_CUDA(cudaFuncSetAttribute(kern, cudaFuncAttributeMaxDynamicSharedMemorySize, WG_SMEM), "o3d_pw_wgrad_tc2");
    const int mt = (Cout + TC_M - 1) / TC_M, nt = (Cin + TC_N - 1) / TC_N;
    const int Mt = mt * TC_M, Nt = nt * TC_N;
    int splits = o3d_num_sms() / (mt * nt);
    if (splits < 1) splits = 1;
    const long long cap = part_floats / ((long long)Mt * Nt);
    if (splits > cap) splits = (int)cap;
    const int by_size = (P + 127) / 128;
    if (splits > by_size) splits = by_size;
    O3D_REQUIRE(splits >= 1, O3D_ERR_ARG, "o3d_pw_wgrad_tc2: workspace too small");
    int chunk = (P + splits - 1) / splits;
    chunk = ((chunk + TC_K - 1) / TC_K) * TC_K;
    splits = (P + chunk - 1) / chunk;
    kern<<<dim3(splits, nt, mt), WG_THREADS, WG_SMEM, st>>>(da, xb, P, Cout, Cin, chunk, part);
    O3D_CHECK_LAUNCH("o3d_pw_wgrad_tc2");
    dim3 rg((Cin / 4 + 31) / 32, Cout);
    wgrad_reduce_kernel<<<rg, 256, 0, st>>>(part, splits, Mt, Nt, Cout, Cin, dw, lddw);
    O3D_CHECK_LAUNCH("o3d_pw_wgrad_tc2: reduce");
    return O3D_OK;
}
inline TcLift make_tclift(const o3d_lift_t* lf, const int32_t* gidx, const float* scale, const float* shift, int relu) {
    return TcLift{LiftView{lf->z, lf->ldz, lf->z ? gidx : nullptr, lf->s, lf->u}, scale, shift, relu, 0};
}
}

extern "C" long long o3d_pw_wgrad_tc2_workspace_floats(void) {
    return (long long)o3d_num_sms() * TC_M * TC_N;
}

int o3d_pw_wgrad_tc2_prec(const float* g, int ldg, const float* y, int ldy, const float* a, const float* b, const float* cc,
                          const float* dpool, const int32_t* sel, int S, int ldp, const float* x, int ldx, const float* in_scale,
                          const float* in_shift, int in_relu, int P, int Cout, int Cin, float* dw, int lddw, float* part,
                          long long part_floats, void* stream, bool bf16) {
    O3D_REQUIRE((g || dpool) && x && dw && part, O3D_ERR_ARG, "o3d_pw_wgrad_tc2: null pointer");
    O3D_REQUIRE((Cout & 3) == 0 && (Cin & 3) == 0 && (ldx & 3) == 0 && (lddw & 3) == 0, O3D_ERR_ARG,
                "o3d_pw_wgrad_tc2: channel counts / leading dimensions must be multiples of 4");
    if (P == 0) return O3D_OK;
    TcDy da{g, ldg, y, ldy, a, b, cc, dpool, sel, S > 0 ? S : 1, ldp, ilog2_exact(S > 0 ? S : 1)};
    TcAct xb{x, ldx, in_scale, in_shift, in_relu};
    if (bf16) return launch_wgrad(da, Bf16<TcAct>{xb}, P, Cout, Cin, dw, lddw, part, part_floats, (cudaStream_t)stream);
    return launch_wgrad(da, xb, P, Cout, Cin, dw, lddw, part, part_floats, (cudaStream_t)stream);
}

extern "C" int o3d_pw_wgrad_tc2(const float* g, int ldg, const float* y, int ldy, const float* a, const float* b,
                                const float* cc, const float* dpool, const int32_t* sel, int S, int ldp, const float* x,
                                int ldx, const float* in_scale, const float* in_shift, int in_relu, int P, int Cout,
                                int Cin, float* dw, int lddw, float* part, long long part_floats, void* stream) {
    return o3d_pw_wgrad_tc2_prec(g, ldg, y, ldy, a, b, cc, dpool, sel, S, ldp, x, ldx, in_scale, in_shift, in_relu, P, Cout, Cin,
                                 dw, lddw, part, part_floats, stream, false);
}

int o3d_pw_wgrad_tc_lift_prec(const float* g, int ldg, const float* y, int ldy, const float* a, const float* b, const float* cc,
                              const float* dpool, const int32_t* sel, int S, int ldp, const o3d_lift_t* lf, const int32_t* gidx,
                              const float* in_scale, const float* in_shift, int in_relu, int P, int Cout, int Cin, float* dw,
                              int lddw, float* part, long long part_floats, void* stream, bool bf16) {
    O3D_REQUIRE((g || dpool) && lf && (gidx || !lf->z) && dw && part, O3D_ERR_ARG, "o3d_pw_wgrad_tc_lift: null pointer");
    O3D_REQUIRE((Cout & 3) == 0 && (Cin & 3) == 0 && lf->ldz == Cin && (lddw & 3) == 0, O3D_ERR_ARG,
                "o3d_pw_wgrad_tc_lift: channel counts / leading dimensions");
    if (P == 0) return O3D_OK;
    TcDy da{g, ldg, y, ldy, a, b, cc, dpool, sel, S > 0 ? S : 1, ldp, ilog2_exact(S > 0 ? S : 1)};
    TcLift xb = make_tclift(lf, gidx, in_scale, in_shift, in_relu);
    xb.la = TC_K;
    if (bf16) return launch_wgrad(da, Bf16<TcLift>{xb}, P, Cout, Cin, dw, lddw, part, part_floats, (cudaStream_t)stream);
    return launch_wgrad(da, xb, P, Cout, Cin, dw, lddw, part, part_floats, (cudaStream_t)stream);
}

extern "C" int o3d_pw_wgrad_tc_lift(const float* g, int ldg, const float* y, int ldy, const float* a, const float* b,
                                    const float* cc, const float* dpool, const int32_t* sel, int S, int ldp,
                                    const o3d_lift_t* lf, const int32_t* gidx, const float* in_scale, const float* in_shift,
                                    int in_relu, int P, int Cout, int Cin, float* dw, int lddw, float* part,
                                    long long part_floats, void* stream) {
    return o3d_pw_wgrad_tc_lift_prec(g, ldg, y, ldy, a, b, cc, dpool, sel, S, ldp, lf, gidx, in_scale, in_shift, in_relu, P, Cout,
                                     Cin, dw, lddw, part, part_floats, stream, false);
}

int o3d_pw_fwd_tc_lift_prec(const o3d_lift_t* lf, const int32_t* gidx, const float* in_scale, const float* in_shift, int in_relu,
                            const void* wtiles, const float* bias, int P, int K, int N, float* y, int ldy, double* sum,
                            double* sumsq, int S, float* ymax, float* ymin, int32_t* arg, int ldp, void* stream, bool bf16) {
    O3D_REQUIRE(lf && (gidx || !lf->z) && wtiles, O3D_ERR_ARG, "o3d_pw_fwd_tc_lift: null pointer");
    O3D_REQUIRE(P >= 0 && K >= 32 && N >= 1 && (K & 3) == 0 && lf->ldz == K, O3D_ERR_ARG, "o3d_pw_fwd_tc_lift: bad sizes");
    O3D_REQUIRE(S == 0 || (P % S == 0 && 64 % S == 0 && ymax && ymin && arg), O3D_ERR_ARG,
                "o3d_pw_fwd_tc_lift: pooling group size must divide 64 and P");
    if (P == 0) return O3D_OK;
    const int Nw = (N + 3) & ~3;
    const TcLift bl = make_tclift(lf, gidx, in_scale, in_shift, in_relu);
    cudaStream_t st = (cudaStream_t)stream;
    if (bf16) {
        const Bf16<TcLift> bb{bl};
#define O3D_FWD_ARGS bb, wtiles, bias, P, K, Nw, y, ldy, sum, sumsq, S, ymax, ymin, arg, ldp, false, st
        if (ldy == 64) return launch_fwd<64>(O3D_FWD_ARGS);
        if (ldy == 128) return launch_fwd<128>(O3D_FWD_ARGS);
        if (ldy == 256) return launch_fwd<256>(O3D_FWD_ARGS);
        return launch_fwd<0>(O3D_FWD_ARGS);
#undef O3D_FWD_ARGS
    }
#define O3D_FWD_ARGS bl, wtiles, bias, P, K, Nw, y, ldy, sum, sumsq, S, ymax, ymin, arg, ldp, false, st
    if (ldy == 64) return launch_fwd<64>(O3D_FWD_ARGS);
    if (ldy == 128) return launch_fwd<128>(O3D_FWD_ARGS);
    if (ldy == 256) return launch_fwd<256>(O3D_FWD_ARGS);
    return launch_fwd<0>(O3D_FWD_ARGS);
#undef O3D_FWD_ARGS
}

extern "C" int o3d_pw_fwd_tc_lift(const o3d_lift_t* lf, const int32_t* gidx, const float* in_scale, const float* in_shift,
                                  int in_relu, const void* wtiles, const float* bias, int P, int K, int N, float* y, int ldy,
                                  double* sum, double* sumsq, int S, float* ymax, float* ymin, int32_t* arg, int ldp,
                                  void* stream) {
    return o3d_pw_fwd_tc_lift_prec(lf, gidx, in_scale, in_shift, in_relu, wtiles, bias, P, K, N, y, ldy, sum, sumsq, S, ymax, ymin,
                                   arg, ldp, stream, false);
}

namespace {
template <class XB, int N>
int launch_bwd(const TcDy& da, const XB& xb, const void* wtiles_t, int P, int M, const TcDgradEpi<N, is_lift<XB>::value>& ep,
               float* dw, int lddw, float* part, long long part_floats, cudaStream_t st) {
    auto kern = pw_bwd_tc_kernel<XB, N>;
    O3D_CUDA(cudaFuncSetAttribute(kern, cudaFuncAttributeMaxDynamicSharedMemorySize, BW_SMEM), "o3d_pw_bwd_tc");
    const int n_ptiles = (P + BW_TP - 1) / BW_TP;
    int gx = o3d_num_sms();
    if (gx > n_ptiles) gx = n_ptiles;
    O3D_REQUIRE(part_floats >= (long long)gx * TC_M * TC_N, O3D_ERR_ARG, "o3d_pw_bwd_tc: workspace too small");
    kern<<<gx, BW_THREADS, BW_SMEM, st>>>(da, xb, (const uint8_t*)wtiles_t, P, M, ep, part);
    O3D_CHECK_LAUNCH("o3d_pw_bwd_tc");
    dim3 rg((N / 4 + 31) / 32, M);
    wgrad_reduce_kernel<<<rg, 256, 0, st>>>(part, gx, TC_M, TC_N, M, N, dw, lddw);
    O3D_CHECK_LAUNCH("o3d_pw_bwd_tc: reduce");
    return O3D_OK;
}

template <class XB>
int bwd_tc_impl(const TcDy& da, const XB& xb, const void* wtiles_t, int P, int Cout, int Cin, float* out, const float* yprev,
                const LiftView* lv, const float* pscale, const float* pshift, int prelu, double* s1, double* s2y, float* dw,
                int lddw, float* part, long long part_floats, cudaStream_t st) {
    constexpr bool LIFT = is_lift<XB>::value;
    auto fill = [&](auto& ep) {
        if constexpr (LIFT) ep.lv = *lv;
        ep.out = out; ep.ldo = Cin; ep.yprev = yprev; ep.ldyp = Cin; ep.scale = pscale; ep.shift = pshift; ep.relu = prelu;
        ep.s1g = s1; ep.s2y = s2y;
    };
    if (Cin == 64) {
        TcDgradEpi<64, LIFT> ep{};
        fill(ep);
        return launch_bwd<XB, 64>(da, xb, wtiles_t, P, Cout, ep, dw, lddw, part, part_floats, st);
    }
    TcDgradEpi<128, LIFT> ep{};
    fill(ep);
    return launch_bwd<XB, 128>(da, xb, wtiles_t, P, Cout, ep, dw, lddw, part, part_floats, st);
}
}

int o3d_pw_bwd_tc_prec(const float* g, int ldg, const float* y, int ldy, const float* a, const float* b, const float* cc,
                       const float* dpool, const int32_t* sel, int S, int ldp, const void* wtiles_t, const float* x,
                       const o3d_lift_t* lf, const int32_t* gidx, const float* in_scale, const float* in_shift, int in_relu, int P,
                       int Cout, int Cin, float* out, double* s1, double* s2y, float* dw, int lddw, float* part,
                       long long part_floats, void* stream, bool bf16) {
    O3D_REQUIRE((g || dpool) && wtiles_t && (x || lf) && out && dw && part, O3D_ERR_ARG, "o3d_pw_bwd_tc: null pointer");
    O3D_REQUIRE((Cout == 64 || Cout == 128) && (Cin == 64 || Cin == 128) && (lddw & 3) == 0, O3D_ERR_ARG,
                "o3d_pw_bwd_tc: channel counts must be 64 or 128");
    O3D_REQUIRE(!lf || ((gidx || !lf->z) && (lf->z || lf->s) && lf->ldz == Cin), O3D_ERR_ARG, "o3d_pw_bwd_tc: lift descriptor");
    if (P == 0) return O3D_OK;
    const TcDy da{g, ldg, y, ldy, a, b, cc, dpool, sel, S > 0 ? S : 1, ldp, ilog2_exact(S > 0 ? S : 1)};
    cudaStream_t st = (cudaStream_t)stream;
    if (lf) {
        TcLift xb = make_tclift(lf, gidx, in_scale, in_shift, in_relu);
        const LiftView lv = xb.lv;
        if (bf16)
            return bwd_tc_impl(da, Bf16<TcLift>{xb}, wtiles_t, P, Cout, Cin, out, nullptr, &lv, in_scale, in_shift, in_relu, s1, s2y,
                               dw, lddw, part, part_floats, st);
        return bwd_tc_impl(da, xb, wtiles_t, P, Cout, Cin, out, nullptr, &lv, in_scale, in_shift, in_relu, s1, s2y, dw, lddw, part,
                           part_floats, st);
    }
    const float* yprev = (in_scale || in_relu) ? x : nullptr;
    const TcAct xb{x, Cin, in_scale, in_shift, in_relu};
    if (bf16)
        return bwd_tc_impl(da, Bf16<TcAct>{xb}, wtiles_t, P, Cout, Cin, out, yprev, nullptr, in_scale, in_shift, in_relu, s1, s2y, dw,
                           lddw, part, part_floats, st);
    return bwd_tc_impl(da, xb, wtiles_t, P, Cout, Cin, out, yprev, nullptr, in_scale, in_shift, in_relu, s1, s2y, dw, lddw, part,
                       part_floats, st);
}

extern "C" int o3d_pw_bwd_tc(const float* g, int ldg, const float* y, int ldy, const float* a, const float* b, const float* cc,
                             const float* dpool, const int32_t* sel, int S, int ldp, const void* wtiles_t, const float* x,
                             const o3d_lift_t* lf, const int32_t* gidx, const float* in_scale, const float* in_shift, int in_relu,
                             int P, int Cout, int Cin, float* out, double* s1, double* s2y, float* dw, int lddw, float* part,
                             long long part_floats, void* stream) {
    return o3d_pw_bwd_tc_prec(g, ldg, y, ldy, a, b, cc, dpool, sel, S, ldp, wtiles_t, x, lf, gidx, in_scale, in_shift, in_relu, P,
                              Cout, Cin, out, s1, s2y, dw, lddw, part, part_floats, stream, false);
}
```

### open3dsot_b200/csrc/stack.cu

```cuda
#include <string.h>
#include "common.cuh"
#include "tc_ptx.cuh"
#include "../../include/o3d_b200.h"

namespace {

inline size_t al(size_t x) { return (x + 255) & ~(size_t)255; }
inline int tc_main(int c) { return c >= 128 ? (c / 128) * 128 : (c >= 64 ? c : 0); }
inline int r4(int x) { return (x + 3) & ~3; }

__device__ __forceinline__ int src_col(int k, int K, int cin, int xyz_first, int c0) {
    if (!xyz_first) return k < cin ? k : -1;
    if (k < c0) return 3 + k;
    if (k >= K - 4 && k < K - 1) return k - (K - 4);
    return -1;
}

__device__ __forceinline__ uint32_t tile_sw128(int r, int c) {
    return (uint32_t)((r >> 3) * 1024 + (r & 7) * 128 + ((c ^ (r & 7)) << 4));
}
__device__ __forceinline__ float tf32_hi(float x) { return __uint_as_float(__float_as_uint(x) & 0xFFFFE000u); }

struct PackLayer {
    const float* src; const float* bias; float* wp; float* wt; float* bias_p; uint8_t* tiles_f; uint8_t* tiles_b;
    int cout, cin, Nw, K, xyz_first, Km , Npad, Kpad ;
};
struct PackArgs { PackLayer l[O3D_MAX_LAYERS]; int c0; int bf16;  };

__global__ void pack_weight_kernel(const PackArgs args) {
    const PackLayer& L = args.l[blockIdx.y];
    const float* __restrict__ src = L.src;
    const float* __restrict__ bias = L.bias;
    float* __restrict__ wp = L.wp;
    float* __restrict__ wt = L.wt;
    float* __restrict__ bias_p = L.bias_p;
    uint8_t* __restrict__ tiles_f = L.tiles_f;
    uint8_t* __restrict__ tiles_b = L.tiles_b;
    const int cout = L.cout, cin = L.cin, Nw = L.Nw, K = L.K, xyz_first = L.xyz_first, c0 = args.c0, Km = L.Km, Npad = L.Npad,
              Kpad = L.Kpad;
    constexpr int TILE = 128 * 32 * 4;
    const int nkb_f = (K + 31) / 32;
    const int k4n = Kpad / 4;
    const int i = blockIdx.x * blockDim.x + threadIdx.x;
    if (bias_p && i < Nw) bias_p[i] = i < cout ? bias[i] : 0.f;
    if (i >= Npad * k4n) return;
    const int n = i / k4n, k = (i % k4n) * 4;
    float v[4] = {0.f, 0.f, 0.f, 0.f};
    if (n < cout) {
#pragma unroll
        for (int j = 0; j < 4; ++j) {
            const int sc = (k + j < K) ? src_col(k + j, K, cin, xyz_first, c0) : -1;
            if (sc >= 0) v[j] = src[(size_t)n * cin + sc];
        }
    }
    if (n < Nw && k < K) {
        *reinterpret_cast<float4*>(wp + (size_t)n * K + k) = make_float4(v[0], v[1], v[2], v[3]);
#pragma unroll
        for (int j = 0; j < 4; ++j) wt[(size_t)(k + j) * Nw + n] = v[j];
    }
    if (tiles_f && k < nkb_f * 32 && args.bf16) {
        uint8_t* dst = tiles_f + ((size_t)(n >> 7) * nkb_f + (k >> 5)) * BF_TILE_BYTES + sw64(n & 127, (k & 31) >> 3) + ((k >> 2) & 1) * 8;
        *reinterpret_cast<uint2*>(dst) = pack_bf16x4(make_float4(v[0], v[1], v[2], v[3]));
    } else if (tiles_f && k < nkb_f * 32) {
        uint8_t* dst = tiles_f + ((size_t)(n >> 7) * nkb_f + (k >> 5)) * (2 * TILE) + tile_sw128(n & 127, (k & 31) >> 2);
        *reinterpret_cast<float4*>(dst) = make_float4(tf32_hi(v[0]), tf32_hi(v[1]), tf32_hi(v[2]), tf32_hi(v[3]));
        *reinterpret_cast<float4*>(dst + TILE) =
            make_float4(v[0] - tf32_hi(v[0]), v[1] - tf32_hi(v[1]), v[2] - tf32_hi(v[2]), v[3] - tf32_hi(v[3]));
    }
    if (tiles_b && n < ((Nw + 31) / 32) * 32) {
        const int nkb_b = (Nw + 31) / 32;
#pragma unroll
        for (int j = 0; j < 4; ++j) {
            const int row = k + j;
            if (row >= ((Km + 127) / 128) * 128) continue;
            const float val = row < Km ? v[j] : 0.f;
            if (args.bf16) {
                uint8_t* dst = tiles_b + ((size_t)(row >> 7) * nkb_b + (n >> 5)) * BF_TILE_BYTES + sw64(row & 127, (n & 31) >> 3) +
                               (n & 7) * 2;
                *reinterpret_cast<uint16_t*>(dst) = (uint16_t)(pack_bf16x2(val, 0.f) & 0xFFFFu);
                continue;
            }
            uint8_t* dst = tiles_b + ((size_t)(row >> 7) * nkb_b + (n >> 5)) * (2 * TILE) + tile_sw128(row & 127, (n & 31) >> 2) +
                           (n & 3) * 4;
            *reinterpret_cast<float*>(dst) = tf32_hi(val);
            *reinterpret_cast<float*>(dst + TILE) = val - tf32_hi(val);
        }
    }
}

struct UnpackLayer { const float* dwp; float* dst; int cout, cin, K, xyz_first; };
struct UnpackArgs { UnpackLayer l[O3D_MAX_LAYERS]; int c0; int accumulate; };

__global__ void unpack_wgrad_kernel(const UnpackArgs args) {
    const UnpackLayer& L = args.l[blockIdx.y];
    const float* __restrict__ dwp = L.dwp;
    float* __restrict__ dst = L.dst;
    const int cout = L.cout, cin = L.cin, K = L.K, xyz_first = L.xyz_first, c0 = args.c0;
    const int i = blockIdx.x * blockDim.x + threadIdx.x;
    if (!dst || i >= cout * K) return;
    const int n = i / K, k = i % K;
    const int sc = src_col(k, K, cin, xyz_first, c0);
    if (sc >= 0) {
        float* o = dst + (size_t)n * cin + sc;
        *o = args.accumulate ? *o + dwp[i] : dwp[i];
    }
}

__global__ void d2f_kernel(const double* __restrict__ src, const float* __restrict__ scale, int n, float* __restrict__ dst,
                           int accumulate) {
    const int i = blockIdx.x * blockDim.x + threadIdx.x;
    if (i < n) dst[i] = (accumulate ? dst[i] : 0.f) + (float)(scale ? src[i] * (double)scale[i] : src[i]);
}

struct Plan {
    int n, P, S, rows;
    bool bf16;
    bool lift, virt;
    size_t gidx;
    int Nw[O3D_MAX_LAYERS], K[O3D_MAX_LAYERS];
    bool tc_f[O3D_MAX_LAYERS], tc_b[O3D_MAX_LAYERS], tc_w[O3D_MAX_LAYERS];
    bool fused_bwd[O3D_MAX_LAYERS];
    size_t wp[O3D_MAX_LAYERS], wt[O3D_MAX_LAYERS], bias[O3D_MAX_LAYERS], y[O3D_MAX_LAYERS], vec[O3D_MAX_LAYERS],
        stat[O3D_MAX_LAYERS], tiles[O3D_MAX_LAYERS];
    size_t ymax, ymin, arg, sel, ysel, stat_all, stat_bytes, fwd_bytes, param_bytes;
    size_t bstat, bstat_bytes, coef[O3D_MAX_LAYERS], dwp[O3D_MAX_LAYERS], btiles[O3D_MAX_LAYERS], dpool, gbuf[2], wpart, bwd_bytes;
    long long wpart_floats;
};

bool make_plan(const o3d_stack_t* d, Plan& p) {
    if (d->n_layers < 1 || d->n_layers > O3D_MAX_LAYERS || d->P < 0 || d->K0 < 4 || (d->K0 & 3)) return false;
    if (d->precision != 0 && !(d->precision == 1 && !d->training) && !(d->precision == 2 && d->training)) return false;
    p.bf16 = d->precision != 0;
    p.n = d->n_layers; p.P = d->P; p.S = d->S;
    p.rows = d->S > 0 ? d->P / d->S : d->P;
    p.lift = d->lift != nullptr;
    p.virt = false;
    if (p.lift && (p.n < 2 || d->weight[0] != nullptr || (d->cout[0] & 3) || d->lift->ldz != d->cout[0] || d->bias[0])) return false;
    size_t o = 0;
    for (int l = 0; l < p.n; ++l) {
        p.Nw[l] = r4(d->cout[l]);
        p.K[l] = l == 0 ? (p.lift ? 0 : d->K0) : p.Nw[l - 1];
        p.tc_f[l] = (d->use_tc & 1) && (p.Nw[l] % 128 == 0 || p.Nw[l] == 64 || !d->training) && p.K[l] >= 32 &&
                    d->P >= (d->training ? O3D_TC_MIN_P_TRAIN : O3D_TC_MIN_P_INFER) &&
                    !(l == d->n_layers - 1 && d->S > 0 && 64 % d->S != 0);
        p.tc_b[l] = (d->use_tc & 1) && p.K[l] >= 64 && p.Nw[l] >= 32 && d->P >= O3D_TC_BWD_MIN_P;
        p.tc_w[l] = (d->use_tc & 2) && p.Nw[l] >= 64 && p.K[l] >= 64 && d->P >= 4096;
    }
    if (p.lift) {
        p.virt = p.tc_f[1] && p.tc_b[1] && (p.tc_w[1] || !d->training) && tc_main(p.K[1]) == p.K[1] && p.K[1] % 32 == 0;
        if (p.virt) p.tc_w[1] = true;
    }
    constexpr int P_FUSED_BWD = 65536;
    for (int l = 0; l < p.n; ++l)
        p.fused_bwd[l] = d->training && p.tc_b[l] && p.tc_w[l] && (p.Nw[l] == 64 || p.Nw[l] == 128) &&
                         (p.K[l] == 64 || p.K[l] == 128) && d->P >= P_FUSED_BWD;
    p.stat_all = o;
    for (int l = 0; l < p.n; ++l) { p.stat[l] = o; o += al(sizeof(double) * 2 * p.Nw[l]); }
    for (int l = 0; l < p.n; ++l) { p.vec[l] = o; o += al(sizeof(float) * 4 * p.Nw[l]); }
    p.stat_bytes = o - p.stat_all;
    for (int l = 0; l < p.n; ++l) {
        p.wp[l] = o; o += al(sizeof(float) * (size_t)p.Nw[l] * p.K[l]);
        p.wt[l] = o; o += al(sizeof(float) * (size_t)p.Nw[l] * p.K[l]);
        p.bias[l] = o; o += al(sizeof(float) * p.Nw[l]);
        p.tiles[l] = o; if (p.tc_f[l]) o += al((size_t)o3d_pw_tc_wtile_bytes(p.Nw[l], p.K[l]) / (p.bf16 ? 4 : 1));
        p.btiles[l] = o; if (p.tc_b[l]) o += al((size_t)o3d_pw_tc_wtile_bytes(tc_main(p.K[l]), p.Nw[l]) / (d->precision == 2 ? 4 : 1));
    }
    p.param_bytes = o;
    for (int l = 0; l < p.n; ++l) {
        p.y[l] = o; if (!(l == 0 && p.virt)) o += al(sizeof(float) * (size_t)p.P * p.Nw[l]);
    }
    p.gidx = o; if (p.lift && d->lift->z) o += al(sizeof(int32_t) * (size_t)p.P);
    const size_t gsz = al(sizeof(float) * (size_t)p.rows * p.Nw[p.n - 1]);
    p.ymax = o; o += p.S > 0 ? gsz : 0;
    p.ymin = o; o += p.S > 0 ? gsz : 0;
    p.arg = o; o += p.S > 0 ? gsz : 0;
    p.sel = o; o += p.S > 0 ? gsz : 0;
    p.ysel = o; o += p.S > 0 ? gsz : 0;
    p.fwd_bytes = o;
    o = 0;
    p.bstat = o;
    for (int l = 0; l < p.n; ++l) o += al(sizeof(double) * 2 * p.Nw[l]);
    size_t maxk = 0;
    for (int l = 0; l < p.n; ++l) { p.coef[l] = o; o += al(sizeof(float) * 5 * p.Nw[l]); }
    for (int l = 0; l < p.n; ++l) { p.dwp[l] = o; o += al(sizeof(float) * (size_t)p.Nw[l] * p.K[l]); }
    p.bstat_bytes = o;
    for (int l = 0; l < p.n; ++l) {
        if ((size_t)p.K[l] > maxk) maxk = p.K[l];
    }
    size_t maxn = 0;
    for (int l = 0; l < p.n; ++l) if ((size_t)p.Nw[l] > maxn) maxn = p.Nw[l];
    if (maxn > maxk) maxk = maxn;
    p.dpool = o; o += p.S > 0 ? gsz : 0;
    for (int i = 0; i < 2; ++i) { p.gbuf[i] = o; o += al(sizeof(float) * (size_t)p.P * maxk); }
    p.wpart = o;
    p.wpart_floats = 0;
    for (int l = 0; l < p.n; ++l)
        if (p.tc_w[l]) p.wpart_floats = o3d_pw_wgrad_tc2_workspace_floats();
    o += al(sizeof(float) * (size_t)p.wpart_floats);
    p.bwd_bytes = o;
    return true;
}

inline double* stat_sum(const Plan& p, uint8_t* ws, int l) { return reinterpret_cast<double*>(ws + p.stat[l]); }
template <class T> inline T* at(uint8_t* ws, size_t off) { return reinterpret_cast<T*>(ws + off); }
template <class T> inline const T* at(const uint8_t* ws, size_t off) { return reinterpret_cast<const T*>(ws + off); }

int pack_params(const o3d_stack_t* d, const Plan& p, uint8_t* ws, int keep_for_backward, cudaStream_t st) {
        PackArgs pa{};
        pa.c0 = d->c0;
        pa.bf16 = p.bf16;
        int work_max = 0;
        for (int l = 0; l < p.n; ++l) {
            const int Nw = p.Nw[l], K = p.K[l];
            PackLayer& q = pa.l[l];
            q.src = d->weight[l]; q.bias = d->bias[l];
            q.wp = at<float>(ws, p.wp[l]); q.wt = at<float>(ws, p.wt[l]);
            q.bias_p = d->bias[l] ? at<float>(ws, p.bias[l]) : nullptr;
            q.tiles_f = p.tc_f[l] ? ws + p.tiles[l] : nullptr;
            q.tiles_b = (p.tc_b[l] && keep_for_backward) ? ws + p.btiles[l] : nullptr;
            q.cout = d->cout[l]; q.cin = d->cin[l]; q.Nw = Nw; q.K = K; q.xyz_first = l == 0 ? d->xyz_first : 0;
            q.Km = tc_main(K);
            q.Npad = Nw; q.Kpad = K;
            if (l == 0 && p.lift) { q.Npad = 0; q.bias_p = nullptr; q.tiles_f = q.tiles_b = nullptr; }
            if (q.tiles_f) { q.Npad = ((Nw + 127) / 128) * 128; q.Kpad = ((K + 31) / 32) * 32; }
            if (q.tiles_b) {
                if (q.Npad < ((Nw + 31) / 32) * 32) q.Npad = ((Nw + 31) / 32) * 32;
                if (q.Kpad < ((q.Km + 127) / 128) * 128) q.Kpad = ((q.Km + 127) / 128) * 128;
            }
            const int work = q.Npad * (q.Kpad / 4);
            if (work > work_max) work_max = work;
        }
        pack_weight_kernel<<<dim3((work_max + 255) / 256, p.n), 256, 0, st>>>(pa);
        O3D_CHECK_LAUNCH("o3d_stack_forward: pack_weight");
    return O3D_OK;
}

}

extern "C" long long o3d_stack_workspace_bytes(const o3d_stack_t* d, int backward) {
    Plan p;
    if (!d || !make_plan(d, p)) return -1;
    return (long long)(backward ? p.bwd_bytes : p.fwd_bytes);
}

extern "C" int o3d_stack_plan_thresholds(const o3d_stack_t* d, int* out) {
    if (!d || !out || d->n_layers < 1 || d->n_layers > O3D_MAX_LAYERS) return -1;
    int n = 0;
    out[n++] = O3D_TC_MIN_P_INFER;
    if (d->lift) out[n++] = O3D_TC_BWD_MIN_P;
    for (int l = d->lift ? 1 : 0; l < d->n_layers; ++l) {
        const int k = l == 0 ? d->K0 : r4(d->cout[l - 1]);
        if (k <= 8 && !(l == d->n_layers - 1 && d->S > 0)) { out[n++] = O3D_FWD_SKINNY_MIN_P; break; }
    }
    return n;
}

extern "C" long long o3d_stack_prepared_bytes(const o3d_stack_t* d) {
    Plan p;
    if (!d || !make_plan(d, p)) return -1;
    return (long long)p.param_bytes;
}

extern "C" int o3d_stack_prepare(const o3d_stack_t* d, void* block, void* stream) {
    O3D_REQUIRE(d && block, O3D_ERR_ARG, "o3d_stack_prepare: null pointer");
    O3D_REQUIRE(!d->training, O3D_ERR_ARG, "o3d_stack_prepare: eval mode only (train-mode BatchNorm needs the batch)");
    Plan p;
    O3D_REQUIRE(make_plan(d, p), O3D_ERR_ARG, "o3d_stack_prepare: bad stack description");
    cudaStream_t st = (cudaStream_t)stream;
    uint8_t* ws = (uint8_t*)block;
    O3D_CUDA(cudaMemsetAsync(ws + p.stat_all, 0, p.stat_bytes, st), "o3d_stack_prepare: memset");
    if (int rc = pack_params(d, p, ws, 0, st)) return rc;
    for (int l = 0; l < p.n; ++l) {
        if (!d->has_bn[l]) continue;
        const int Nw = p.Nw[l];
        float* vec = at<float>(ws, p.vec[l]);
        if (int rc = o3d_bn_fwd_finalize(nullptr, nullptr, (double)p.P, d->gamma[l], d->beta[l], d->running_mean[l], d->running_var[l],
                                         nullptr, d->momentum[l], d->eps[l], 0, d->cout[l], vec, vec + Nw, vec + 2 * Nw, vec + 3 * Nw,
                                         stream))
            return rc;
    }
    return O3D_OK;
}

extern "C" int o3d_stack_forward(const o3d_stack_t* d, const float* x, void* ws_fwd, float* out, int keep_for_backward,
                                 void* stream) {
    O3D_REQUIRE(d && (x || d->lift) && ws_fwd && out, O3D_ERR_ARG, "o3d_stack_forward: null pointer");
    O3D_REQUIRE(d->precision == 0 || (d->precision == 1 && d->prepared && !d->training && !keep_for_backward) ||
                    (d->precision == 2 && d->training),
                O3D_ERR_ARG, "o3d_stack_forward: precision %d needs inference on a prepared block (precision 1: no training, no "
                "keep_for_backward) or training (precision 2)", d->precision);
    Plan p;
    O3D_REQUIRE(make_plan(d, p), O3D_ERR_ARG, "o3d_stack_forward: bad stack description");
    O3D_REQUIRE(p.S == 0 || (128 % p.S == 0 && p.P % p.S == 0), O3D_ERR_ARG, "o3d_stack_forward: group size %d", p.S);
    if (p.P == 0) return O3D_OK;
    cudaStream_t st = (cudaStream_t)stream;
    uint8_t* ws = (uint8_t*)ws_fwd;
    const bool prepared = d->prepared != nullptr;
    O3D_REQUIRE(!prepared || (!d->training && !keep_for_backward), O3D_ERR_ARG, "o3d_stack_forward: a prepared block is for inference only");
    uint8_t* wsp = prepared ? (uint8_t*)d->prepared : ws;
    if (!prepared) {
        O3D_CUDA(cudaMemsetAsync(ws + p.stat_all, 0, p.stat_bytes, st), "o3d_stack_forward: memset");
        if (int rc = pack_params(d, p, wsp, keep_for_backward, st)) return rc;
    }
    const float* cur = x;
    int cur_ld = d->K0;
    const float *in_scale = nullptr, *in_shift = nullptr;
    int in_relu = 0;
    const int L = p.n - 1;
    for (int l = 0; l < p.n; ++l) {
        const int Nw = p.Nw[l], K = p.K[l], cout = d->cout[l];
        float* wt = at<float>(wsp, p.wt[l]);
        float* bias = d->bias[l] ? at<float>(wsp, p.bias[l]) : nullptr;
        const bool last = l == L, pool = last && p.S > 0;
        const bool keep_y = !last || keep_for_backward || !pool;
        float* y = keep_y ? at<float>(ws, p.y[l]) : nullptr;
        const bool stats = d->training && d->has_bn[l];
        double* sum = stats ? stat_sum(p, wsp, l) : nullptr;
        double* sumsq = stats ? sum + Nw : nullptr;
        float* ymax = pool ? at<float>(ws, p.ymax) : nullptr;
        float* ymin = pool ? at<float>(ws, p.ymin) : nullptr;
        int32_t* arg = pool ? at<int32_t>(ws, p.arg) : nullptr;
        int rc;
        if (l == 0 && p.lift) {
            rc = o3d_lift_stats(d->lift, p.P, Nw, at<int32_t>(ws, p.gidx), p.virt ? nullptr : y, sum, sumsq, stream);
        } else if (l == 1 && p.virt) {
            rc = o3d_pw_fwd_tc_lift_prec(d->lift, at<int32_t>(ws, p.gidx), in_scale, in_shift, in_relu, wsp + p.tiles[l], bias, p.P,
                                         K, cout, y, Nw, sum, sumsq, pool ? p.S : 0, ymax, ymin, arg, Nw, stream, p.bf16);
        } else if (p.tc_f[l]) {
            void* tiles = wsp + p.tiles[l];
            rc = o3d_pw_fwd_tc_dir(cur, cur_ld, in_scale, in_shift, in_relu, tiles, bias, p.P, K, cout, y, Nw, sum, sumsq,
                                   pool ? p.S : 0, ymax, ymin, arg, Nw, stream, (l & 1) == 0, p.bf16);
        } else {
            rc = o3d_pw_fwd(cur, cur_ld, in_scale, in_shift, in_relu, wt, Nw, bias, p.P, K, cout, y, Nw, sum, sumsq,
                            pool ? p.S : 0, ymax, ymin, arg, Nw, stream);
        }
        if (rc) return rc;
        float* vec = at<float>(wsp, p.vec[l]);
        float *sc = nullptr, *sh = nullptr;
        if (d->has_bn[l]) {
            sc = vec; sh = vec + Nw;
            if (!prepared)
            rc = o3d_bn_fwd_finalize(sum, sumsq, (double)p.P, d->gamma[l], d->beta[l], d->running_mean[l], d->running_var[l],
                                     d->training ? d->num_batches_tracked[l] : nullptr, d->momentum[l], d->eps[l],
                                     d->training, cout, sc, sh, vec + 2 * Nw, vec + 3 * Nw, stream);
            if (rc) return rc;
        }
        if (last) {
            if (pool) {
                rc = o3d_pool_finalize(ymax, ymin, arg, sc, sh, d->relu[l], p.rows, Nw, Nw, out, Nw,
                                       keep_for_backward ? at<int32_t>(ws, p.sel) : nullptr,
                                       keep_for_backward ? at<float>(ws, p.ysel) : nullptr, stream);
            } else if (d->has_bn[l] || d->relu[l]) {
                rc = o3d_act_apply(y, Nw, sc, sh, d->relu[l], p.P, Nw, out, Nw, stream);
            } else {
                O3D_CUDA(cudaMemcpyAsync(out, y, sizeof(float) * (size_t)p.P * Nw, cudaMemcpyDeviceToDevice, st),
                         "o3d_stack_forward: copy out");
                rc = O3D_OK;
            }
            if (rc) return rc;
        }
        cur = y; cur_ld = Nw; in_scale = sc; in_shift = sh; in_relu = d->relu[l];
    }
    return O3D_OK;
}

extern "C" int o3d_stack_backward(const o3d_stack_t* d, const float* x, const void* ws_fwd, void* ws_bwd, const float* out,
                                  const float* dout, float* dx, void* stream) {
    O3D_REQUIRE(d && (x || d->lift) && ws_fwd && ws_bwd && out && dout, O3D_ERR_ARG, "o3d_stack_backward: null pointer");
    O3D_REQUIRE(d->precision == 0 || d->precision == 2, O3D_ERR_ARG, "o3d_stack_backward: precision %d is for inference only",
                d->precision);
    Plan p;
    O3D_REQUIRE(make_plan(d, p), O3D_ERR_ARG, "o3d_stack_backward: bad stack description");
    if (p.P == 0) return O3D_OK;
    cudaStream_t st = (cudaStream_t)stream;
    const uint8_t* wf = (const uint8_t*)ws_fwd;
    uint8_t* wb = (uint8_t*)ws_bwd;
    O3D_CUDA(cudaMemsetAsync(wb + p.bstat, 0, p.bstat_bytes, st), "o3d_stack_backward: memset");
    auto s1 = [&](int l) { size_t o = p.bstat; for (int i = 0; i < l; ++i) o += al(sizeof(double) * 2 * p.Nw[i]); return at<double>(wb, o); };
    const int L = p.n - 1;
    const int NwL = p.Nw[L];
    const float* yL = at<float>(wf, p.y[L]);
    const float* g = nullptr;
    float* dpool = nullptr;
    int rc;
    if (p.S > 0) {
        dpool = at<float>(wb, p.dpool);
        rc = o3d_pool_bwd_prep(dout, NwL, out, NwL, at<float>(wf, p.ysel), d->relu[L], p.rows, NwL, NwL, dpool, s1(L),
                               s1(L) + NwL, stream);
        if (rc) return rc;
    } else if (d->has_bn[L] || d->relu[L]) {
        float* gb = at<float>(wb, p.gbuf[0]);
        rc = o3d_dense_bwd_prep(dout, NwL, out, NwL, yL, NwL, d->relu[L], p.P, NwL, gb, NwL, s1(L), s1(L) + NwL, stream);
        if (rc) return rc;
        g = gb;
    } else {
        g = dout;
        if (d->bias[L]) {
            rc = o3d_dense_bwd_prep(dout, NwL, nullptr, 0, nullptr, 0, 0, p.P, NwL, nullptr, 0, s1(L), nullptr, stream);
            if (rc) return rc;
        }
    }
    int gsel = (g == at<float>(wb, p.gbuf[0])) ? 1 : 0;
    for (int l = L; l >= 0; --l) {
        const int Nl = p.Nw[l], K = p.K[l], cout = d->cout[l];
        float* coef = at<float>(wb, p.coef[l]);
        const float *a = nullptr, *b = nullptr, *cc = nullptr;
        const float* vec = at<float>(wf, p.vec[l]);
        if (d->has_bn[l]) {
            rc = o3d_bn_bwd_finalize(s1(l), s1(l) + Nl, (double)p.P, d->gamma[l], vec + 2 * Nl, vec + 3 * Nl,
                                     (d->training ? 1 : 0) | (d->accumulate ? 2 : 0),
                                     cout, coef, coef + Nl, coef + 2 * Nl, d->d_gamma[l], d->d_beta[l], stream);
            if (rc) return rc;
            a = coef; b = coef + Nl; cc = coef + 2 * Nl;
            if (d->d_bias[l] && d->training) {
                if (!d->accumulate)
                    O3D_CUDA(cudaMemsetAsync(d->d_bias[l], 0, sizeof(float) * cout, st), "d_bias");
            } else if (d->d_bias[l]) {
                d2f_kernel<<<(cout + 127) / 128, 128, 0, st>>>(s1(l), a, cout, d->d_bias[l], d->accumulate);
            }
        } else if (d->d_bias[l]) {
            d2f_kernel<<<(cout + 127) / 128, 128, 0, st>>>(s1(l), nullptr, cout, d->d_bias[l], d->accumulate);
        }
        if (l == 0 && p.lift) {
            const o3d_lift_t* lf = d->lift;
            if (lf->d_z || lf->d_s || lf->d_u) {
                rc = o3d_lift_scatter(lf, p.P, Nl, at<int32_t>(wf, p.gidx), p.virt ? nullptr : at<float>(wf, p.y[0]), g, Nl, a, b,
                                      cc, stream);
                if (rc) return rc;
            }
            break;
        }
        const bool pooled = (l == L && p.S > 0);
        const float* gl = pooled ? nullptr : g;
        const float* yl = a ? at<float>(wf, p.y[l]) : nullptr;
        const float* dpl = pooled ? dpool : nullptr;
        const int32_t* sel = pooled ? at<int32_t>(wf, p.sel) : nullptr;
        const int Sg = pooled ? p.S : 0;
        const float* xin = l == 0 ? x : at<float>(wf, p.y[l - 1]);
        const float* pvec = l == 0 ? nullptr : at<float>(wf, p.vec[l - 1]);
        const int Kp = K;
        const float* psc = (l > 0 && d->has_bn[l - 1]) ? pvec : nullptr;
        const float* psh = (l > 0 && d->has_bn[l - 1]) ? pvec + Kp : nullptr;
        const int prelu = l > 0 ? d->relu[l - 1] : 0;
        if (p.fused_bwd[l] && (l > 0 || dx) && d->d_weight[l]) {
            float* gout = l > 0 ? at<float>(wb, p.gbuf[gsel]) : dx;
            const bool want = l > 0 && (d->has_bn[l - 1] || d->bias[l - 1] != nullptr);
            const bool lifted = l == 1 && p.virt;
            rc = o3d_pw_bwd_tc_prec(gl, Nl, yl, Nl, a, b, cc, dpl, sel, Sg, Nl, wf + p.btiles[l], lifted ? nullptr : xin,
                                    lifted ? d->lift : nullptr, lifted ? at<int32_t>(wf, p.gidx) : nullptr, psc, psh, prelu, p.P, Nl,
                                    K, gout, want ? s1(l - 1) : nullptr, want ? s1(l - 1) + K : nullptr, at<float>(wb, p.dwp[l]), K,
                                    at<float>(wb, p.wpart), p.wpart_floats, stream, p.bf16);
            if (rc) return rc;
            g = gout;
            gsel ^= 1;
            continue;
        }
        if (l > 0 || dx) {
            float* gout = l > 0 ? at<float>(wb, p.gbuf[gsel]) : dx;
            const bool mask = l > 0 && (d->has_bn[l - 1] || d->relu[l - 1]);
            const bool want = l > 0 && (d->has_bn[l - 1] || d->bias[l - 1] != nullptr);
            const float* yprev = mask ? at<float>(wf, p.y[l - 1]) : nullptr;
            double* ps1 = want ? s1(l - 1) : nullptr;
            double* ps2 = want ? s1(l - 1) + K : nullptr;
            if (l == 1 && p.virt) {
                rc = o3d_pw_dgrad_tc_lift_prec(gl, Nl, yl, Nl, a, b, cc, dpl, sel, Sg, Nl, wf + p.btiles[l], p.P, Nl, K, gout, K,
                                               d->lift, at<int32_t>(wf, p.gidx), psc, psh, prelu, ps1, ps2, stream, p.bf16);
            } else if (p.tc_b[l]) {
                const int Km = tc_main(K);
                const void* tiles = wf + p.btiles[l];
                rc = o3d_pw_dgrad_tc_prec(gl, Nl, yl, Nl, a, b, cc, dpl, sel, Sg, Nl, tiles, p.P, Nl, Km, gout, K, yprev, K, psc, psh,
                                          prelu, ps1, ps2, stream, p.bf16);
                if (rc) return rc;
                const bool tail_wanted = !(l == 0 && d->dx_cols > 0 && d->dx_cols <= Km);
                if (K > Km && tail_wanted)
                    rc = o3d_pw_dgrad(gl, Nl, yl, Nl, a, b, cc, dpl, sel, Sg, Nl, at<float>(wf, p.wp[l]) + Km, K, p.P, Nl, K - Km,
                                      gout + Km, K, yprev ? yprev + Km : nullptr, K, psc ? psc + Km : nullptr,
                                      psh ? psh + Km : nullptr, prelu, ps1 ? ps1 + Km : nullptr, ps2 ? ps2 + Km : nullptr, stream);
            } else {
                rc = o3d_pw_dgrad(gl, Nl, yl, Nl, a, b, cc, dpl, sel, Sg, Nl, at<float>(wf, p.wp[l]), K, p.P, Nl, K, gout, K,
                                  yprev, K, psc, psh, prelu, ps1, ps2, stream);
            }
            if (rc) return rc;
            g = gout;
            gsel ^= 1;
        }
        if (d->d_weight[l]) {
            float* dwp = at<float>(wb, p.dwp[l]);
            if (l == 1 && p.virt) {
                rc = o3d_pw_wgrad_tc_lift_prec(gl, Nl, yl, Nl, a, b, cc, dpl, sel, Sg, Nl, d->lift, at<int32_t>(wf, p.gidx), psc, psh,
                                               prelu, p.P, Nl, K, dwp, K, at<float>(wb, p.wpart), p.wpart_floats, stream, p.bf16);
            } else if (p.tc_w[l]) {
                const int Kmain = tc_main(K);
                rc = o3d_pw_wgrad_tc2_prec(gl, Nl, yl, Nl, a, b, cc, dpl, sel, Sg, Nl, xin, K, psc, psh, prelu, p.P, Nl, Kmain, dwp,
                                           K, at<float>(wb, p.wpart), p.wpart_floats, stream, p.bf16);
                if (rc) return rc;
                if (K > Kmain)
                    rc = o3d_pw_wgrad(gl, Nl, yl, Nl, a, b, cc, dpl, sel, Sg, Nl, xin + Kmain, K, psc ? psc + Kmain : nullptr,
                                      psh ? psh + Kmain : nullptr, prelu, p.P, Nl, K - Kmain, dwp + Kmain, K, stream);
            } else {
                rc = o3d_pw_wgrad(gl, Nl, yl, Nl, a, b, cc, dpl, sel, Sg, Nl, xin, K, psc, psh, prelu, p.P, Nl, K, dwp, K, stream);
            }
            if (rc) return rc;
        }
    }
    {
        UnpackArgs ua{};
        ua.c0 = d->c0;
        ua.accumulate = d->accumulate;
        int work_max = 0;
        for (int l = 0; l < p.n; ++l) {
            UnpackLayer& q = ua.l[l];
            q.dwp = at<float>(wb, p.dwp[l]); q.dst = d->d_weight[l];
            q.cout = d->cout[l]; q.cin = d->cin[l]; q.K = p.K[l]; q.xyz_first = l == 0 ? d->xyz_first : 0;
            if (q.dst && q.cout * q.K > work_max) work_max = q.cout * q.K;
        }
        if (work_max > 0) {
            unpack_wgrad_kernel<<<dim3((work_max + 255) / 256, p.n), 256, 0, st>>>(ua);
            O3D_CHECK_LAUNCH("o3d_stack_backward: unpack_wgrad");
        }
    }
    return O3D_OK;
}
```

Baseline: 3011.

## Reduce lifted-layer gradients per row inside dgrad epilogue instead of materialising per-point gradients

Adds a row mode for the virtual lifted first layer. The layer-1 dgrad epilogue accumulates the input gradient directly into per-row sums (run-length atomics over sorted gather indices) and per-block partials for the u-gradient, so the per-point gradient buffer is never written. A new finish step counts rows, then converts the row sums into dz and du with the BN coefficients applied. The goal is to avoid writing and re-reading a P×C gradient tensor and the separate scatter pass, at the cost of atomics in the epilogue, extra workspace, and an added rowcount kernel.

```diff
diff --git a/open3dsot_b200/csrc/common.cuh b/open3dsot_b200/csrc/common.cuh
--- a/open3dsot_b200/csrc/common.cuh
+++ b/open3dsot_b200/csrc/common.cuh
@@ -153,6 +153,7 @@
                       const float* bias, int P, int K, int N, float* y, int ldy, double* sum, double* sumsq, int S, float* ymax,
                       float* ymin, int32_t* arg, int ldp, void* stream, bool reverse, bool bf16);
 struct o3d_lift_t;
+struct LiftRows;
 int o3d_pw_fwd_tc_lift_prec(const o3d_lift_t* lf, const int32_t* gidx, const float* in_scale, const float* in_shift, int in_relu,
                             const void* wtiles, const float* bias, int P, int K, int N, float* y, int ldy, double* sum,
                             double* sumsq, int S, float* ymax, float* ymin, int32_t* arg, int ldp, void* stream, bool bf16);
@@ -163,7 +164,8 @@
 int o3d_pw_dgrad_tc_lift_prec(const float* g, int ldg, const float* y, int ldy, const float* a, const float* b, const float* cc,
                               const float* dpool, const int32_t* sel, int S, int ldp, const void* wtiles_t, int P, int Cout,
                               int Cin, float* out, int ldo, const o3d_lift_t* lf, const int32_t* gidx, const float* pscale,
-                              const float* pshift, int prelu, double* s1, double* s2y, void* stream, bool bf16);
+                              const float* pshift, int prelu, double* s1, double* s2y, void* stream, bool bf16,
+                              const LiftRows* rows);
 int o3d_pw_wgrad_tc2_prec(const float* g, int ldg, const float* y, int ldy, const float* a, const float* b, const float* cc,
                           const float* dpool, const int32_t* sel, int S, int ldp, const float* x, int ldx, const float* in_scale,
                           const float* in_shift, int in_relu, int P, int Cout, int Cin, float* dw, int lddw, float* part,
@@ -176,6 +178,10 @@
                        const float* dpool, const int32_t* sel, int S, int ldp, const void* wtiles_t, const float* x,
                        const o3d_lift_t* lf, const int32_t* gidx, const float* in_scale, const float* in_shift, int in_relu, int P,
                        int Cout, int Cin, float* out, double* s1, double* s2y, float* dw, int lddw, float* part,
-                       long long part_floats, void* stream, bool bf16);
+                       long long part_floats, void* stream, bool bf16, const LiftRows* rows);
+long long o3d_lift_rows_slots();
+int lift_rows_check(const o3d_lift_t* lf, const LiftRows* rows, int C0, const char* who);
+int o3d_lift_finish(const o3d_lift_t* lf, int P, int C0, const int32_t* gidx, int zrows, const LiftRows* rows, const float* a,
+                    const float* b, const float* cc, void* stream);
 
 #endif
diff --git a/open3dsot_b200/csrc/lift.cu b/open3dsot_b200/csrc/lift.cu
--- a/open3dsot_b200/csrc/lift.cu
+++ b/open3dsot_b200/csrc/lift.cu
@@ -80,11 +80,130 @@
     }
 }
 
+constexpr int LIFT_ROWCOUNT_RUN = 4;
+__global__ void __launch_bounds__(LIFT_THREADS)
+    lift_rowcount_kernel(LiftView lv, int P, float* __restrict__ rcnt, float4* __restrict__ rsum) {
+    const int n_chunks = (P + LIFT_ROWCOUNT_RUN - 1) / LIFT_ROWCOUNT_RUN;
+    for (int ci = blockIdx.x * blockDim.x + threadIdx.x; ci < n_chunks; ci += gridDim.x * blockDim.x) {
+        const int pb = ci * LIFT_ROWCOUNT_RUN, pe = min(pb + LIFT_ROWCOUNT_RUN, P);
+        int row = __ldg(lv.gidx + pb);
+        float cnt = 0.f;
+        float4 sr = make_float4(0.f, 0.f, 0.f, 0.f);
+        for (int p = pb; p < pe; ++p) {
+            const int rk = __ldg(lv.gidx + p);
+            if (rk != row) {
+                atomicAdd(rcnt + row, cnt);
+                if (rsum) atomicAdd(rsum + row, sr);
+                row = rk; cnt = 0.f; sr = make_float4(0.f, 0.f, 0.f, 0.f);
+            }
+            cnt += 1.f;
+            if (rsum) { const float4 sv = ldg4(lv.s + (size_t)p * 4); sr.x += sv.x; sr.y += sv.y; sr.z += sv.z; sr.w += sv.w; }
+        }
+        atomicAdd(rcnt + row, cnt);
+        if (rsum) atomicAdd(rsum + row, sr);
+    }
+}
+
+__device__ __forceinline__ void rows_dz(const LiftView& lv, const LiftRows& lr, int zrows, int C0, const float* ca, const float* cb,
+                                        const float* ccf, float* __restrict__ dz, float* __restrict__ du, float* red) {
+    const int tpr = C0 >> 2, rl = blockDim.x / tpr;
+    const int t = threadIdx.x % tpr, lane = threadIdx.x / tpr;
+    const int c = t * 4;
+    const U4 u = load_u(lv, c);
+    const float4 zero = make_float4(0.f, 0.f, 0.f, 0.f);
+    const float4 a4 = ca ? ldg4(ca + c) : zero, b4 = cb ? ldg4(cb + c) : zero, k4 = ccf ? ldg4(ccf + c) : zero;
+    const bool wz = du && ccf && lr.rsum;
+    if (blockIdx.x * rl >= zrows) return;
+    float4 w0 = zero, w1 = zero, w2 = zero, w3 = zero;
+    for (int r = blockIdx.x * rl + lane; r < zrows; r += gridDim.x * rl) {
+        const size_t o = (size_t)r * lv.ldz + c;
+        const float4 S = lr.rsum ? __ldg(lr.rsum + r) : zero;
+        const float4 zr = ldg4(lv.z + o);
+        if (dz) {
+            float4 d = ldg4(lr.gsum + o);
+            if (ca) {
+                const float n = __ldg(lr.rcnt + r);
+                const float4 h = lift_val4(make_float4(n * zr.x, n * zr.y, n * zr.z, n * zr.w), S, u.u0, u.u1, u.u2, u.u3);
+                d.x = fmaf(a4.x, d.x, fmaf(k4.x, h.x, n * b4.x)); d.y = fmaf(a4.y, d.y, fmaf(k4.y, h.y, n * b4.y));
+                d.z = fmaf(a4.z, d.z, fmaf(k4.z, h.z, n * b4.z)); d.w = fmaf(a4.w, d.w, fmaf(k4.w, h.w, n * b4.w));
+            }
+            float4* q = reinterpret_cast<float4*>(dz + o);
+            float4 v = *q;
+            v.x += d.x; v.y += d.y; v.z += d.z; v.w += d.w;
+            *q = v;
+        }
+        if (wz) {
+            w0.x = fmaf(S.x, zr.x, w0.x); w0.y = fmaf(S.x, zr.y, w0.y); w0.z = fmaf(S.x, zr.z, w0.z); w0.w = fmaf(S.x, zr.w, w0.w);
+            w1.x = fmaf(S.y, zr.x, w1.x); w1.y = fmaf(S.y, zr.y, w1.y); w1.z = fmaf(S.y, zr.z, w1.z); w1.w = fmaf(S.y, zr.w, w1.w);
+            w2.x = fmaf(S.z, zr.x, w2.x); w2.y = fmaf(S.z, zr.y, w2.y); w2.z = fmaf(S.z, zr.z, w2.z); w2.w = fmaf(S.z, zr.w, w2.w);
+            w3.x = fmaf(S.w, zr.x, w3.x); w3.y = fmaf(S.w, zr.y, w3.y); w3.z = fmaf(S.w, zr.z, w3.z); w3.w = fmaf(S.w, zr.w, w3.w);
+        }
+    }
+    if (!wz) return;
+    float* rr = red + (size_t)lane * 4 * C0 + c;
+    *reinterpret_cast<float4*>(rr) = w0;
+    *reinterpret_cast<float4*>(rr + C0) = w1;
+    *reinterpret_cast<float4*>(rr + 2 * C0) = w2;
+    *reinterpret_cast<float4*>(rr + 3 * C0) = w3;
+    __syncthreads();
+    for (int e = threadIdx.x; e < 4 * C0; e += blockDim.x) {
+        float s1 = 0.f;
+        for (int l = 0; l < rl; ++l) s1 += red[(size_t)l * 4 * C0 + e];
+        atomicAdd(du + e, __ldg(ccf + e % C0) * s1);
+    }
+}
+
+__device__ __forceinline__ void rows_du(const LiftView& lv, const LiftRows& lr, int C0, const float* ca, const float* cb,
+                                        const float* ccf, float* __restrict__ du) {
+    const int sub = threadIdx.x & 7;
+    const int e = blockIdx.x * (blockDim.x >> 3) + (threadIdx.x >> 3);
+    if (blockIdx.x * (blockDim.x >> 3) >= 4 * C0) return;
+    const bool on = e < 4 * C0;
+    const int j = on ? e / C0 : 0, c = on ? e % C0 : 0;
+    int qc[4];
+#pragma unroll
+    for (int i = 0; i < 4; ++i) qc[i] = lift_pair_index(min(i, j), max(i, j));
+    float A = 0.f, Ss = 0.f, Q[4] = {0.f, 0.f, 0.f, 0.f};
+    if (on)
+        for (int s = sub; s < lr.nslot; s += 8) {
+            const float* base = lr.part + (size_t)s * LIFT_PART_ROWS * C0;
+            A += __ldg(base + (size_t)j * C0 + c);
+            Ss += __ldg(base + (size_t)4 * C0 + j);
+#pragma unroll
+            for (int i = 0; i < 4; ++i) Q[i] += __ldg(base + (size_t)4 * C0 + qc[i]);
+        }
+    const int w0 = threadIdx.x & ~31;
+    const unsigned m = blockDim.x - w0 >= 32 ? 0xFFFFFFFFu : (1u << (blockDim.x - w0)) - 1u;
+#pragma unroll
+    for (int o = 4; o >= 1; o >>= 1) {
+        A += __shfl_xor_sync(m, A, o); Ss += __shfl_xor_sync(m, Ss, o);
+#pragma unroll
+        for (int i = 0; i < 4; ++i) Q[i] += __shfl_xor_sync(m, Q[i], o);
+    }
+    if (sub != 0 || !on) return;
+    float r = A;
+    if (ca) {
+        float t = 0.f;
+        if (cb) {
+            const float y = fmaf(Q[3], __ldg(lv.u + 3 * C0 + c), fmaf(Q[2], __ldg(lv.u + 2 * C0 + c),
+                                 fmaf(Q[1], __ldg(lv.u + C0 + c), Q[0] * __ldg(lv.u + c))));
+            t = fmaf(__ldg(cb + c), Ss, __ldg(ccf + c) * y);
+        }
+        r = fmaf(__ldg(ca + c), A, t);
+    }
+    du[e] += r;
+}
+
 __global__ void __launch_bounds__(LIFT_THREADS, 4)
     lift_scatter_kernel(LiftView lv, int P, int C0, int grp, const float* __restrict__ y0, const float* __restrict__ g, int ldg,
                         const float* __restrict__ ca, const float* __restrict__ cb, const float* __restrict__ ccf,
-                        float* __restrict__ dz, float* __restrict__ ds, float* __restrict__ du) {
+                        float* __restrict__ dz, float* __restrict__ ds, float* __restrict__ du, LiftRows lr, int zrows) {
     extern __shared__ float redf[];
+    if (lr.nslot > 0) {
+        if (blockIdx.y == 0) { if (lv.z) rows_dz(lv, lr, zrows, C0, ca, cb, ccf, dz, du, redf); }
+        else if (du) rows_du(lv, lr, C0, ca, cb, ccf, du);
+        return;
+    }
     const int tpr = C0 >> 2, rl = blockDim.x / tpr;
     const int t = threadIdx.x % tpr, lane = threadIdx.x / tpr;
     const int c = t * 4;
@@ -220,7 +339,55 @@
     const size_t smem = (lf->s && lf->d_u) ? sizeof(float) * rl * 4 * C0 : 0;
     lift_scatter_kernel<<<blocks, threads, smem, (cudaStream_t)stream>>>(lv, P, C0, lf->grp, y0, g, ldg, a, b, cc,
                                                                         lf->z ? lf->d_z : nullptr, lf->s ? lf->d_s : nullptr,
-                                                                        lf->s ? lf->d_u : nullptr);
+                                                                        lf->s ? lf->d_u : nullptr, LiftRows{}, 0);
     O3D_CHECK_LAUNCH("o3d_lift_scatter");
     return O3D_OK;
 }
+
+long long o3d_lift_rows_slots() { return 4LL * o3d_num_sms(); }
+
+int lift_rows_check(const o3d_lift_t* lf, const LiftRows* rows, int C0, const char* who) {
+    if (!rows) return O3D_OK;
+    O3D_REQUIRE(rows->nslot >= o3d_lift_rows_slots() && C0 % 32 == 0, O3D_ERR_ARG,
+                "%s: row mode needs %lld partial slots (got %d) and C0 %% 32 == 0 (C0 = %d)", who, o3d_lift_rows_slots(),
+                rows->nslot, C0);
+    O3D_REQUIRE(!lf->d_s, O3D_ERR_ARG, "%s: row mode is for a lift without d_s", who);
+    O3D_REQUIRE((!lf->s || (lf->u && rows->part)) && (!lf->z || (rows->gsum && rows->rcnt && (!lf->s || rows->rsum))), O3D_ERR_ARG,
+                "%s: row-mode buffers missing", who);
+    O3D_REQUIRE(((uintptr_t)rows->gsum & 15) == 0 && ((uintptr_t)rows->rsum & 15) == 0, O3D_ERR_ALIGN,
+                "%s: row-mode buffers must be 16-byte aligned", who);
+    return O3D_OK;
+}
+
+int o3d_lift_finish(const o3d_lift_t* lf, int P, int C0, const int32_t* gidx, int zrows, const LiftRows* rows, const float* a,
+                    const float* b, const float* cc, void* stream) {
+    if (int e = lift_check(lf, P, C0, "o3d_lift_finish")) return e;
+    O3D_REQUIRE(rows && (gidx || !lf->z) && zrows >= 0, O3D_ERR_ARG, "o3d_lift_finish: null pointer / zrows");
+    if (int e = lift_rows_check(lf, rows, C0, "o3d_lift_finish")) return e;
+    O3D_REQUIRE(!b == !cc, O3D_ERR_ARG, "o3d_lift_finish: b and cc come together");
+    O3D_REQUIRE(((uintptr_t)lf->d_z & 15) == 0, O3D_ERR_ALIGN, "o3d_lift_finish: alignment");
+    float* dz = lf->z ? lf->d_z : nullptr;
+    float* du = lf->s ? lf->d_u : nullptr;
+    if (P == 0 || (!dz && !du)) return O3D_OK;
+    cudaStream_t st = (cudaStream_t)stream;
+    const LiftView lv = make_view(lf, gidx);
+    int threads, blocks, rl;
+    lift_launch_shape(P, C0, lf->grp, threads, blocks, rl);
+    int rb = 0;
+    if (lf->z) {
+        const int nc = (P + LIFT_ROWCOUNT_RUN - 1) / LIFT_ROWCOUNT_RUN;
+        int cb = (nc + LIFT_THREADS - 1) / LIFT_THREADS;
+        if (cb > 16 * o3d_num_sms()) cb = 16 * o3d_num_sms();
+        lift_rowcount_kernel<<<cb, LIFT_THREADS, 0, st>>>(lv, P, rows->rcnt, lf->s ? rows->rsum : nullptr);
+        O3D_CHECK_LAUNCH("o3d_lift_finish: rowcount");
+        rb = (zrows + rl - 1) / rl;
+        if (rb > 8 * o3d_num_sms()) rb = 8 * o3d_num_sms();
+    }
+    const int ub = du ? (4 * C0 + threads / 8 - 1) / (threads / 8) : 0;
+    blocks = rb > ub ? rb : ub;
+    const size_t smem = (lf->z && du) ? sizeof(float) * rl * 4 * C0 : 0;
+    lift_scatter_kernel<<<dim3(blocks, 2), threads, smem, st>>>(lv, P, C0, lf->grp, nullptr, nullptr, 0, a, b, cc, dz, nullptr, du,
+                                                               *rows, zrows);
+    O3D_CHECK_LAUNCH("o3d_lift_finish");
+    return O3D_OK;
+}
diff --git a/open3dsot_b200/csrc/lift.cuh b/open3dsot_b200/csrc/lift.cuh
--- a/open3dsot_b200/csrc/lift.cuh
+++ b/open3dsot_b200/csrc/lift.cuh
@@ -1,5 +1,6 @@
 #pragma once
 #include <stdint.h>
+#include <vector_types.h>
 
 struct LiftView {
     const float* z; int ldz;
@@ -7,6 +8,16 @@
     const float* s;
     const float* u;
 };
+
+struct LiftRows {
+    float* gsum;
+    float* rcnt;
+    float4* rsum;
+    float* part;
+    int nslot;
+};
+constexpr int LIFT_PART_ROWS = 5;
+inline __host__ __device__ int lift_pair_index(int i, int j) { return 4 + i * 4 - i * (i - 1) / 2 + (j - i); }
 
 #ifdef __CUDACC__
 __device__ __forceinline__ float lift_val(float z, const float4& s, float u0, float u1, float u2, float u3) {
diff --git a/open3dsot_b200/csrc/pwmlp_tc.cu b/open3dsot_b200/csrc/pwmlp_tc.cu
--- a/open3dsot_b200/csrc/pwmlp_tc.cu
+++ b/open3dsot_b200/csrc/pwmlp_tc.cu
@@ -207,7 +207,7 @@
     float* y; int ldy; const float* bias; double* sum; double* sumsq;
     int S, log2S; float* ymax; float* ymin; int32_t* arg; int ldp;
     float bv, mx, mn; int ax, an; double d1, d2;
-    __device__ __forceinline__ void begin(int ch, int Nw) {
+    __device__ __forceinline__ void begin(int ch, int Nw, int, float*) {
         d1 = d2 = 0.0;
         bv = (bias && ch < Nw) ? bias[ch] : 0.f;
         mx = -INFINITY; mn = INFINITY; ax = an = 0;
@@ -290,11 +290,13 @@
     float* out; int ldo; const float* yprev; int ldyp; const float* scale; const float* shift; int relu;
     double* s1g; double* s2y;
     LiftView lv;
+    LiftRows lr;
     float sc, sh; double d1, d2;
     float yv[16];
     float u0, u1, u2, u3; const int32_t* gs; const float4* ss;
+    float* racc; int slot;
     __device__ __forceinline__ bool lifted() const { return LIFT; }
-    __device__ __forceinline__ void begin(int ch, int Nw) {
+    __device__ __forceinline__ void begin(int ch, int Nw, int slot_, float* racc_) {
         d1 = d2 = 0.0;
         sc = (scale && ch < Nw) ? scale[ch] : 1.f;
         sh = (shift && ch < Nw) ? shift[ch] : 0.f;
@@ -302,6 +304,10 @@
             const bool on = lv.u && ch < Nw;
             u0 = on ? lv.u[ch] : 0.f; u1 = on ? lv.u[lv.ldz + ch] : 0.f; u2 = on ? lv.u[2 * lv.ldz + ch] : 0.f; u3 = on ? lv.u[3 * lv.ldz + ch] : 0.f;
             gs = nullptr;
+            slot = slot_;
+            racc = racc_;
+#pragma unroll
+            for (int i = 0; i < LIFT_PART_ROWS; ++i) racc[i * 256] = 0.f;
         }
     }
     __device__ __forceinline__ const int32_t* lift_gidx() const { return LIFT ? lv.gidx : nullptr; }
@@ -332,8 +338,67 @@
             }
         }
     }
+    __device__ __forceinline__ void group_rows(const uint32_t (&r)[16], int ch, int pbase, int P) {
+        const int n = min(16, P - pbase);
+        if (n <= 0) return;
+        const int col = pbase & (TC_N - 1);
+        float v[16];
+        float s1 = 0.f, s2 = 0.f;
+#pragma unroll
+        for (int j = 0; j < 16; ++j) {
+            v[j] = j < n ? __uint_as_float(r[j]) : 0.f;
+            if (relu) v[j] = fmaf(yv[j], sc, sh) > 0.f ? v[j] : 0.f;
+        }
+#pragma unroll
+        for (int j = 0; j < 16; ++j) s2 = fmaf(v[j], yv[j], s2);
+#pragma unroll
+        for (int j = 0; j < 16; ++j) s1 += v[j];
+        d1 += (double)s1;
+        d2 += (double)s2;
+        if (lv.z) {
+            int row = gs[col];
+            float run = 0.f;
+#pragma unroll
+            for (int j = 0; j < 16; ++j) {
+                if (j < n) {
+                    const int rj = gs[col + j];
+                    if (rj != row) { atomicAdd(lr.gsum + (size_t)row * lv.ldz + ch, run); row = rj; run = 0.f; }
+                    run += v[j];
+                }
+            }
+            atomicAdd(lr.gsum + (size_t)row * lv.ldz + ch, run);
+        }
+        if (!lv.s) return;
+        float a0 = 0.f, a1 = 0.f, a2 = 0.f, a3 = 0.f;
+#pragma unroll
+        for (int j = 0; j < 16; ++j) {
+            const float4 s = j < n ? ss[col + j] : make_float4(0.f, 0.f, 0.f, 0.f);
+            a0 = fmaf(s.x, v[j], a0); a1 = fmaf(s.y, v[j], a1); a2 = fmaf(s.z, v[j], a2); a3 = fmaf(s.w, v[j], a3);
+        }
+        racc[0] += a0; racc[256] += a1; racc[512] += a2; racc[768] += a3;
+        if (ch < 32) {
+            const int lane = ch, k = lane % 14, k4 = k - 4, hf = lane / 14;
+            const int qi = k < 4 ? k : k4 < 4 ? 0 : k4 < 7 ? 1 : k4 < 9 ? 2 : 3;
+            const int qj = k < 4 ? 4 : k4 < 4 ? k4 : k4 < 7 ? k4 - 3 : k4 < 9 ? k4 - 5 : 3;
+            float q = 0.f;
+            if (hf < 2) {
+#pragma unroll
+                for (int j = 0; j < 8; ++j) {
+                    if (8 * hf + j < n) {
+                        const float* sp = reinterpret_cast<const float*>(ss + col + 8 * hf + j);
+                        q = fmaf(sp[qi], qj < 4 ? sp[qj] : 1.f, q);
+                    }
+                }
+            }
+            q += __shfl_down_sync(0xFFFFFFFFu, q, 14);
+            if (lane < 14) racc[1024] += q;
+        }
+    }
     __device__ __forceinline__ void group(const uint32_t (&r)[16], int ch, int Nw, int pbase, int P) {
         if (ch >= Nw) return;
+        if constexpr (LIFT) {
+            if (lr.nslot > 0) { group_rows(r, ch, pbase, P); return; }
+        }
         float s1 = 0.f, s2 = 0.f;
         float* op = out + (size_t)pbase * ldo + ch;
         if (pbase + 16 <= P) {
@@ -375,6 +440,14 @@
             atomicAdd(s1g + ch, d1);
             atomicAdd(s2y + ch, d2);
         }
+        if constexpr (LIFT) {
+            if (lr.nslot > 0 && lr.part && ch < Nw) {
+                float* o = lr.part + (size_t)slot * LIFT_PART_ROWS * lv.ldz + ch;
+#pragma unroll
+                for (int i = 0; i < 4; ++i) o[(size_t)i * lv.ldz] = racc[i * 256];
+                if (ch < 14) o[(size_t)4 * lv.ldz] = racc[4 * 256];
+            }
+        }
     }
 };
 
@@ -383,7 +456,8 @@
 constexpr int TC_EPI_LD = 68;
 constexpr int TC_EPI_BYTES = TC_M * TC_EPI_LD * 4;
 constexpr int TC_THREADS = 512;
-constexpr int TC_SMEM = TC_STAGES * TC_STAGE_BYTES + 2 * TC_EPI_BYTES + 1024 + 256 + 1024 + 4096;
+constexpr int LIFT_RACC_OFF = 256 + 1024 + 4096, LIFT_RACC_BYTES = LIFT_PART_ROWS * 256 * 4;
+constexpr int TC_SMEM = TC_STAGES * TC_STAGE_BYTES + 2 * TC_EPI_BYTES + 1024 + LIFT_RACC_OFF + LIFT_RACC_BYTES;
 
 template <int R>
 __device__ __forceinline__ void stage_acc(const float (&acc)[R], float* stg, int ld) {
@@ -427,7 +501,7 @@
         float* stg = reinterpret_cast<float*>(smem + TC_STAGES * TC_STAGE_BYTES + h * TC_EPI_BYTES);
         int32_t* gsm = reinterpret_cast<int32_t*>(tail + 256);
         float4* ssm = reinterpret_cast<float4*>(tail + 256 + 1024);
-        epi.begin(ch, Nw);
+        epi.begin(ch, Nw, blockIdx.x * 2 + h, reinterpret_cast<float*>(tail + LIFT_RACC_OFF) + threadIdx.x);
         int stage = 0, phase = 0, buf = 0;
         for (int t = blockIdx.x; t < n_ptiles; t += gridDim.x) {
             const int pt0 = tile_of(t) * TC_N;
@@ -707,7 +781,7 @@
 constexpr int BW_TP = 64;
 constexpr int BW_THREADS = 384;
 constexpr int BW_DY = 0, BW_XT = 64 * 1024, BW_W = 128 * 1024, BW_TAIL = 192 * 1024;
-constexpr int BW_SMEM = BW_TAIL + 256 + 1024 + 4096 + 1024;
+constexpr int BW_SMEM = BW_TAIL + LIFT_RACC_OFF + LIFT_RACC_BYTES + 1024;
 constexpr int BW_BF_SUB = BW_TP * TC_BF_ROW;
 
 template <class XB, int N>
@@ -768,7 +842,7 @@
         float* stg = reinterpret_cast<float*>(smem + BW_XT + h * (NH * TC_EPI_LD * 4));
         int32_t* gsm = reinterpret_cast<int32_t*>(tail + 256);
         float4* ssm = reinterpret_cast<float4*>(tail + 256 + 1024);
-        epi.begin(n_local, N);
+        epi.begin(n_local, N, blockIdx.x * (256 / N) + q, reinterpret_cast<float*>(tail + LIFT_RACC_OFF) + threadIdx.x);
         float wacc[N / 2];
 #pragma unroll
         for (int i = 0; i < N / 2; ++i) wacc[i] = 0.f;
@@ -1009,12 +1083,13 @@
 template <int LD, bool LIFT = false, class BL>
 int launch_dgrad(const BL& bl, const void* wtiles_t, int P, int Cout, int Cin, float* out, int ldo, const float* yprev,
                  int ldyp, const float* pscale, const float* pshift, int prelu, double* s1, double* s2y, cudaStream_t st,
-                 const LiftView* lv = nullptr) {
+                 const LiftView* lv = nullptr, const LiftRows* lr = nullptr) {
     if constexpr (!LIFT) {
-        if (lv) return launch_dgrad<LD, true>(bl, wtiles_t, P, Cout, Cin, out, ldo, yprev, ldyp, pscale, pshift, prelu, s1, s2y, st, lv);
+        if (lv) return launch_dgrad<LD, true>(bl, wtiles_t, P, Cout, Cin, out, ldo, yprev, ldyp, pscale, pshift, prelu, s1, s2y, st, lv, lr);
     }
     TcDgradEpi<LD, LIFT> ep{};
     if (lv) ep.lv = *lv;
+    if (lr) ep.lr = *lr;
     ep.out = out; ep.ldo = ldo; ep.yprev = yprev; ep.ldyp = ldyp; ep.scale = pscale; ep.shift = pshift; ep.relu = prelu;
     ep.s1g = s1; ep.s2y = s2y;
     return launch_tc(bl, (const uint8_t*)wtiles_t, P, Cout, Cin, ep, false, st, "o3d_pw_dgrad_tc");
@@ -1076,15 +1151,15 @@
 int dgrad_tc_impl(const float* g, int ldg, const float* y, int ldy, const float* a, const float* b, const float* cc,
                   const float* dpool, const int32_t* sel, int S, int ldp, const void* wtiles_t, int P, int Cout, int Cin,
                   float* out, int ldo, const float* yprev, int ldyp, const float* pscale, const float* pshift, int prelu,
-                  double* s1, double* s2y, void* stream, const LiftView* lv, bool bf16) {
-    O3D_REQUIRE((g || dpool) && wtiles_t && out, O3D_ERR_ARG, "o3d_pw_dgrad_tc: null pointer");
+                  double* s1, double* s2y, void* stream, const LiftView* lv, const LiftRows* lr, bool bf16) {
+    O3D_REQUIRE((g || dpool) && wtiles_t && (out || lr), O3D_ERR_ARG, "o3d_pw_dgrad_tc: null pointer");
     O3D_REQUIRE((Cout & 3) == 0 && (Cin & 3) == 0, O3D_ERR_ARG, "o3d_pw_dgrad_tc: channel counts must be multiples of 4");
     if (P == 0) return O3D_OK;
     TcDy bl{g, ldg, y, ldy, a, b, cc, dpool, sel, S > 0 ? S : 1, ldp, ilog2_exact(S > 0 ? S : 1)};
     cudaStream_t st = (cudaStream_t)stream;
     const int ld = (!yprev || ldyp == ldo) ? ldo : 0;
     auto run = [&](const auto& ldr) {
-#define O3D_DG_ARGS ldr, wtiles_t, P, Cout, Cin, out, ldo, yprev, ldyp, pscale, pshift, prelu, s1, s2y, st, lv
+#define O3D_DG_ARGS ldr, wtiles_t, P, Cout, Cin, out, ldo, yprev, ldyp, pscale, pshift, prelu, s1, s2y, st, lv, lr
         if (ld == 64) return launch_dgrad<64>(O3D_DG_ARGS);
         if (ld == 128) return launch_dgrad<128>(O3D_DG_ARGS);
         if (ld == 256) return launch_dgrad<256>(O3D_DG_ARGS);
@@ -1100,7 +1175,7 @@
                          float* out, int ldo, const float* yprev, int ldyp, const float* pscale, const float* pshift, int prelu,
                          double* s1, double* s2y, void* stream, bool bf16) {
     return dgrad_tc_impl(g, ldg, y, ldy, a, b, cc, dpool, sel, S, ldp, wtiles_t, P, Cout, Cin, out, ldo, yprev, ldyp, pscale,
-                         pshift, prelu, s1, s2y, stream, nullptr, bf16);
+                         pshift, prelu, s1, s2y, stream, nullptr, nullptr, bf16);
 }
 
 extern "C" int o3d_pw_dgrad_tc(const float* g, int ldg, const float* y, int ldy, const float* a, const float* b,
@@ -1109,17 +1184,19 @@
                                int ldyp, const float* pscale, const float* pshift, int prelu, double* s1, double* s2y,
                                void* stream) {
     return dgrad_tc_impl(g, ldg, y, ldy, a, b, cc, dpool, sel, S, ldp, wtiles_t, P, Cout, Cin, out, ldo, yprev, ldyp, pscale,
-                         pshift, prelu, s1, s2y, stream, nullptr, false);
+                         pshift, prelu, s1, s2y, stream, nullptr, nullptr, false);
 }
 
 int o3d_pw_dgrad_tc_lift_prec(const float* g, int ldg, const float* y, int ldy, const float* a, const float* b, const float* cc,
                               const float* dpool, const int32_t* sel, int S, int ldp, const void* wtiles_t, int P, int Cout,
                               int Cin, float* out, int ldo, const o3d_lift_t* lf, const int32_t* gidx, const float* pscale,
-                              const float* pshift, int prelu, double* s1, double* s2y, void* stream, bool bf16) {
+                              const float* pshift, int prelu, double* s1, double* s2y, void* stream, bool bf16,
+                              const LiftRows* rows) {
     O3D_REQUIRE(lf && (gidx || !lf->z) && (lf->z || lf->s) && lf->ldz == Cin, O3D_ERR_ARG, "o3d_pw_dgrad_tc_lift: lift descriptor");
+    if (int e = lift_rows_check(lf, rows, Cin, "o3d_pw_dgrad_tc_lift")) return e;
     const LiftView lv{lf->z, lf->ldz, lf->z ? gidx : nullptr, lf->s, lf->u};
     return dgrad_tc_impl(g, ldg, y, ldy, a, b, cc, dpool, sel, S, ldp, wtiles_t, P, Cout, Cin, out, ldo, nullptr, 0, pscale,
-                         pshift, prelu, s1, s2y, stream, &lv, bf16);
+                         pshift, prelu, s1, s2y, stream, &lv, rows, bf16);
 }
 
 extern "C" int o3d_pw_dgrad_tc_lift(const float* g, int ldg, const float* y, int ldy, const float* a, const float* b,
@@ -1128,7 +1205,7 @@
                                     const o3d_lift_t* lf, const int32_t* gidx, const float* pscale, const float* pshift,
                                     int prelu, double* s1, double* s2y, void* stream) {
     return o3d_pw_dgrad_tc_lift_prec(g, ldg, y, ldy, a, b, cc, dpool, sel, S, ldp, wtiles_t, P, Cout, Cin, out, ldo, lf, gidx, pscale,
-                                     pshift, prelu, s1, s2y, stream, false);
+                                     pshift, prelu, s1, s2y, stream, false, nullptr);
 }
 
 namespace {
@@ -1267,11 +1344,14 @@
 
 template <class XB>
 int bwd_tc_impl(const TcDy& da, const XB& xb, const void* wtiles_t, int P, int Cout, int Cin, float* out, const float* yprev,
-                const LiftView* lv, const float* pscale, const float* pshift, int prelu, double* s1, double* s2y, float* dw,
-                int lddw, float* part, long long part_floats, cudaStream_t st) {
+                const LiftView* lv, const LiftRows* lr, const float* pscale, const float* pshift, int prelu, double* s1, double* s2y,
+                float* dw, int lddw, float* part, long long part_floats, cudaStream_t st) {
     constexpr bool LIFT = is_lift<XB>::value;
     auto fill = [&](auto& ep) {
-        if constexpr (LIFT) ep.lv = *lv;
+        if constexpr (LIFT) {
+            ep.lv = *lv;
+            if (lr) ep.lr = *lr;
+        }
         ep.out = out; ep.ldo = Cin; ep.yprev = yprev; ep.ldyp = Cin; ep.scale = pscale; ep.shift = pshift; ep.relu = prelu;
         ep.s1g = s1; ep.s2y = s2y;
     };
@@ -1290,11 +1370,14 @@
                        const float* dpool, const int32_t* sel, int S, int ldp, const void* wtiles_t, const float* x,
                        const o3d_lift_t* lf, const int32_t* gidx, const float* in_scale, const float* in_shift, int in_relu, int P,
                        int Cout, int Cin, float* out, double* s1, double* s2y, float* dw, int lddw, float* part,
-                       long long part_floats, void* stream, bool bf16) {
-    O3D_REQUIRE((g || dpool) && wtiles_t && (x || lf) && out && dw && part, O3D_ERR_ARG, "o3d_pw_bwd_tc: null pointer");
+                       long long part_floats, void* stream, bool bf16, const LiftRows* rows) {
+    O3D_REQUIRE((g || dpool) && wtiles_t && (x || lf) && (out || rows) && dw && part, O3D_ERR_ARG, "o3d_pw_bwd_tc: null pointer");
     O3D_REQUIRE((Cout == 64 || Cout == 128) && (Cin == 64 || Cin == 128) && (lddw & 3) == 0, O3D_ERR_ARG,
                 "o3d_pw_bwd_tc: channel counts must be 64 or 128");
     O3D_REQUIRE(!lf || ((gidx || !lf->z) && (lf->z || lf->s) && lf->ldz == Cin), O3D_ERR_ARG, "o3d_pw_bwd_tc: lift descriptor");
+    O3D_REQUIRE(!rows || lf, O3D_ERR_ARG, "o3d_pw_bwd_tc: row mode needs a lifted input");
+    if (rows)
+        if (int e = lift_rows_check(lf, rows, Cin, "o3d_pw_bwd_tc")) return e;
     if (P == 0) return O3D_OK;
     const TcDy da{g, ldg, y, ldy, a, b, cc, dpool, sel, S > 0 ? S : 1, ldp, ilog2_exact(S > 0 ? S : 1)};
     cudaStream_t st = (cudaStream_t)stream;
@@ -1302,18 +1385,18 @@
         TcLift xb = make_tclift(lf, gidx, in_scale, in_shift, in_relu);
         const LiftView lv = xb.lv;
         if (bf16)
-            return bwd_tc_impl(da, Bf16<TcLift>{xb}, wtiles_t, P, Cout, Cin, out, nullptr, &lv, in_scale, in_shift, in_relu, s1, s2y,
-                               dw, lddw, part, part_floats, st);
-        return bwd_tc_impl(da, xb, wtiles_t, P, Cout, Cin, out, nullptr, &lv, in_scale, in_shift, in_relu, s1, s2y, dw, lddw, part,
-                           part_floats, st);
+            return bwd_tc_impl(da, Bf16<TcLift>{xb}, wtiles_t, P, Cout, Cin, out, nullptr, &lv, rows, in_scale, in_shift, in_relu, s1,
+                               s2y, dw, lddw, part, part_floats, st);
+        return bwd_tc_impl(da, xb, wtiles_t, P, Cout, Cin, out, nullptr, &lv, rows, in_scale, in_shift, in_relu, s1, s2y, dw, lddw,
+                           part, part_floats, st);
     }
     const float* yprev = (in_scale || in_relu) ? x : nullptr;
     const TcAct xb{x, Cin, in_scale, in_shift, in_relu};
     if (bf16)
-        return bwd_tc_impl(da, Bf16<TcAct>{xb}, wtiles_t, P, Cout, Cin, out, yprev, nullptr, in_scale, in_shift, in_relu, s1, s2y, dw,
-                           lddw, part, part_floats, st);
-    return bwd_tc_impl(da, xb, wtiles_t, P, Cout, Cin, out, yprev, nullptr, in_scale, in_shift, in_relu, s1, s2y, dw, lddw, part,
-                       part_floats, st);
+        return bwd_tc_impl(da, Bf16<TcAct>{xb}, wtiles_t, P, Cout, Cin, out, yprev, nullptr, nullptr, in_scale, in_shift, in_relu, s1,
+                           s2y, dw, lddw, part, part_floats, st);
+    return bwd_tc_impl(da, xb, wtiles_t, P, Cout, Cin, out, yprev, nullptr, nullptr, in_scale, in_shift, in_relu, s1, s2y, dw, lddw,
+                       part, part_floats, st);
 }
 
 extern "C" int o3d_pw_bwd_tc(const float* g, int ldg, const float* y, int ldy, const float* a, const float* b, const float* cc,
@@ -1322,5 +1405,5 @@
                              int P, int Cout, int Cin, float* out, double* s1, double* s2y, float* dw, int lddw, float* part,
                              long long part_floats, void* stream) {
     return o3d_pw_bwd_tc_prec(g, ldg, y, ldy, a, b, cc, dpool, sel, S, ldp, wtiles_t, x, lf, gidx, in_scale, in_shift, in_relu, P,
-                              Cout, Cin, out, s1, s2y, dw, lddw, part, part_floats, stream, false);
-}
+                              Cout, Cin, out, s1, s2y, dw, lddw, part, part_floats, stream, false, nullptr);
+}
diff --git a/open3dsot_b200/csrc/stack.cu b/open3dsot_b200/csrc/stack.cu
--- a/open3dsot_b200/csrc/stack.cu
+++ b/open3dsot_b200/csrc/stack.cu
@@ -1,6 +1,7 @@
 #include <string.h>
 #include "common.cuh"
 #include "tc_ptx.cuh"
+#include "lift.cuh"
 #include "../../include/o3d_b200.h"
 
 namespace {
@@ -124,6 +125,8 @@
         stat[O3D_MAX_LAYERS], tiles[O3D_MAX_LAYERS];
     size_t ymax, ymin, arg, sel, ysel, stat_all, stat_bytes, fwd_bytes, param_bytes;
     size_t bstat, bstat_bytes, coef[O3D_MAX_LAYERS], dwp[O3D_MAX_LAYERS], btiles[O3D_MAX_LAYERS], dpool, gbuf[2], wpart, bwd_bytes;
+    size_t lr_g, lr_n, lr_s, lr_part;
+    int lrows_n, zrows;
     long long wpart_floats;
 };
 
@@ -183,6 +186,14 @@
     size_t maxk = 0;
     for (int l = 0; l < p.n; ++l) { p.coef[l] = o; o += al(sizeof(float) * 5 * p.Nw[l]); }
     for (int l = 0; l < p.n; ++l) { p.dwp[l] = o; o += al(sizeof(float) * (size_t)p.Nw[l] * p.K[l]); }
+    const bool rmode = p.virt && p.Nw[0] % 32 == 0;
+    const o3d_lift_t* lf = d->lift;
+    p.zrows = (rmode && lf->z) ? (p.P / lf->pos_per_cloud) * lf->rows_per_cloud : 0;
+    p.lrows_n = rmode ? (int)o3d_lift_rows_slots() : 0;
+    p.lr_g = o; o += al(sizeof(float) * (size_t)p.zrows * p.Nw[0]);
+    p.lr_n = o; o += al(sizeof(float) * (size_t)p.zrows);
+    p.lr_s = o; o += (rmode && lf->s) ? al(sizeof(float) * 4 * (size_t)p.zrows) : 0;
+    p.lr_part = o; o += (rmode && lf->s) ? al(sizeof(float) * (size_t)p.lrows_n * LIFT_PART_ROWS * p.Nw[0]) : 0;
     p.bstat_bytes = o;
     for (int l = 0; l < p.n; ++l) {
         if ((size_t)p.K[l] > maxk) maxk = p.K[l];
@@ -401,6 +412,13 @@
         }
     }
     int gsel = (g == at<float>(wb, p.gbuf[0])) ? 1 : 0;
+    LiftRows lrows{};
+    if (p.lrows_n > 0 && !d->lift->d_s) {
+        const o3d_lift_t* lf = d->lift;
+        lrows = LiftRows{lf->z ? at<float>(wb, p.lr_g) : nullptr, lf->z ? at<float>(wb, p.lr_n) : nullptr,
+                         (lf->z && lf->s) ? at<float4>(wb, p.lr_s) : nullptr, lf->s ? at<float>(wb, p.lr_part) : nullptr, p.lrows_n};
+    }
+    const LiftRows* rows = lrows.nslot > 0 ? &lrows : nullptr;
     for (int l = L; l >= 0; --l) {
         const int Nl = p.Nw[l], K = p.K[l], cout = d->cout[l];
         float* coef = at<float>(wb, p.coef[l]);
@@ -423,7 +441,11 @@
         }
         if (l == 0 && p.lift) {
             const o3d_lift_t* lf = d->lift;
-            if (lf->d_z || lf->d_s || lf->d_u) {
+            if (rows) {
+                rc = o3d_lift_finish(lf, p.P, Nl, at<int32_t>(wf, p.gidx), p.zrows, rows, a, d->training ? b : nullptr,
+                                     d->training ? cc : nullptr, stream);
+                if (rc) return rc;
+            } else if (lf->d_z || lf->d_s || lf->d_u) {
                 rc = o3d_lift_scatter(lf, p.P, Nl, at<int32_t>(wf, p.gidx), p.virt ? nullptr : at<float>(wf, p.y[0]), g, Nl, a, b,
                                       cc, stream);
                 if (rc) return rc;
@@ -443,20 +465,20 @@
         const float* psh = (l > 0 && d->has_bn[l - 1]) ? pvec + Kp : nullptr;
         const int prelu = l > 0 ? d->relu[l - 1] : 0;
         if (p.fused_bwd[l] && (l > 0 || dx) && d->d_weight[l]) {
-            float* gout = l > 0 ? at<float>(wb, p.gbuf[gsel]) : dx;
+            const bool lifted = l == 1 && p.virt;
+            float* gout = (lifted && rows) ? nullptr : l > 0 ? at<float>(wb, p.gbuf[gsel]) : dx;
             const bool want = l > 0 && (d->has_bn[l - 1] || d->bias[l - 1] != nullptr);
-            const bool lifted = l == 1 && p.virt;
             rc = o3d_pw_bwd_tc_prec(gl, Nl, yl, Nl, a, b, cc, dpl, sel, Sg, Nl, wf + p.btiles[l], lifted ? nullptr : xin,
                                     lifted ? d->lift : nullptr, lifted ? at<int32_t>(wf, p.gidx) : nullptr, psc, psh, prelu, p.P, Nl,
                                     K, gout, want ? s1(l - 1) : nullptr, want ? s1(l - 1) + K : nullptr, at<float>(wb, p.dwp[l]), K,
-                                    at<float>(wb, p.wpart), p.wpart_floats, stream, p.bf16);
+                                    at<float>(wb, p.wpart), p.wpart_floats, stream, p.bf16, lifted ? rows : nullptr);
             if (rc) return rc;
             g = gout;
             gsel ^= 1;
             continue;
         }
         if (l > 0 || dx) {
-            float* gout = l > 0 ? at<float>(wb, p.gbuf[gsel]) : dx;
+            float* gout = (l == 1 && p.virt && rows) ? nullptr : l > 0 ? at<float>(wb, p.gbuf[gsel]) : dx;
             const bool mask = l > 0 && (d->has_bn[l - 1] || d->relu[l - 1]);
             const bool want = l > 0 && (d->has_bn[l - 1] || d->bias[l - 1] != nullptr);
             const float* yprev = mask ? at<float>(wf, p.y[l - 1]) : nullptr;
@@ -464,7 +486,7 @@
             double* ps2 = want ? s1(l - 1) + K : nullptr;
             if (l == 1 && p.virt) {
                 rc = o3d_pw_dgrad_tc_lift_prec(gl, Nl, yl, Nl, a, b, cc, dpl, sel, Sg, Nl, wf + p.btiles[l], p.P, Nl, K, gout, K,
-                                               d->lift, at<int32_t>(wf, p.gidx), psc, psh, prelu, ps1, ps2, stream, p.bf16);
+                                               d->lift, at<int32_t>(wf, p.gidx), psc, psh, prelu, ps1, ps2, stream, p.bf16, rows);
             } else if (p.tc_b[l]) {
                 const int Km = tc_main(K);
                 const void* tiles = wf + p.btiles[l];
```

Result: faster. 3067, median of 6 (+1.9%).
